# browserdotsys/vecchio

Measured on NVIDIA B200. Metric: Mpaths/s, higher is better.
Workload: dtype f32

## Files before the change

### include/vecchio_gpu.h

```cpp
#ifndef VECCHIO_GPU_H
#define VECCHIO_GPU_H

#include <stddef.h>
#include <stdint.h>

#ifdef __cplusplus
extern "C" {
#endif

#define VK_API_VERSION 1u

typedef enum vk_status {
    VK_OK = 0,
    VK_ERR_INVALID = -1,
    VK_ERR_NO_DEVICE = -2,
    VK_ERR_CUDA = -3,
    VK_ERR_UNSUPPORTED = -4,
    VK_ERR_NO_SCENE = -5,
    VK_ERR_OOM = -6
} vk_status;


typedef uint32_t vk_ref;

// ... 135 lines not shown
    float origin[3];
    float lower_left_corner[3];
    float horizontal[3];
    float vertical[3];
    float u[3], v[3], w[3];
    float lens_radius;
    float time0, time1;
} vk_camera;

enum { VK_VARIANT_AUTO = 0, VK_VARIANT_MEGAKERNEL = 1, VK_VARIANT_WAVEFRONT = 2, VK_VARIANT_STAGED = 3, VK_VARIANT_WARPQ = 4,
       VK_VARIANT_STEPQ = 5 };
enum {
    VK_FLAG_STRICT_MATH = 1u,
    VK_FLAG_FORCE_BVH = 2u,
    VK_FLAG_LEGACY_SCATTER = 4u,
    VK_FLAG_SKY_BACKGROUND = 8u
};

typedef struct vk_render_params {
    uint32_t width, height;
    uint32_t spp;
    uint32_t spp_begin;
    uint32_t spp_count;
    uint32_t max_depth;
    uint64_t seed;
    float background[3];
    uint32_t variant;
    uint32_t flags;
} vk_render_params;

typedef struct vk_stats {
    uint64_t paths;
    uint64_t rays;
    uint64_t dropped_samples;
    float ms_kernels;
    float ms_total;
    uint32_t variant;
    uint32_t launches;
    uint64_t node_visits;
    uint64_t prim_tests;
} vk_stats;

typedef struct vk_ray {
    float origin[3];
    float direction[3];
    float time;
    float tmin, tmax;
} vk_ray;

typedef struct vk_hit {
    vk_ref prim;
    uint32_t face;
    uint32_t mat;
    uint32_t front;
    float t;
    float p[3];
    float normal[3];
    float u, v;
    uint32_t _pad;
} vk_hit;

#define VK_MEDIUM_XI_SLOTS 8

typedef struct vk_ctx vk_ctx;

int vk_create(int device, vk_ctx** out);
void vk_destroy(vk_ctx* ctx);
const char* vk_last_error(const vk_ctx* ctx);

int vk_scene_upload(vk_ctx* ctx, const vk_scene_desc* scene);

typedef struct vk_scene_info {
    uint32_t flat_entries;
    uint32_t flat_segments;
    uint32_t flat_subtrees;
    uint32_t simple;
    uint32_t wide_nodes;
    uint32_t wide_levels_world;
    uint32_t wide_levels_instance;
    uint32_t stack_need;
    uint32_t dynamic_megakernel;
    uint32_t flat_boxes;
    uint32_t flat_direct;
} vk_scene_info;
int vk_scene_check(const vk_scene_desc* scene, vk_scene_info* info, char* err, size_t err_len);

int vk_render(vk_ctx* ctx, const vk_camera* cam, const vk_render_params* params,
              float* out_rgb, float* out_sumsq, vk_stats* stats);

int vk_render_rgb8(vk_ctx* ctx, const vk_camera* cam, const vk_render_params* params,
                   uint8_t* out_rgb8, vk_stats* stats);

int vk_render_frames(vk_ctx* ctx, const vk_camera* cams, uint32_t n_frames, const vk_render_params* params,
                     float* out_rgb, vk_stats* stats);
int vk_render_frames_rgb8(vk_ctx* ctx, const vk_camera* cams, uint32_t n_frames, const vk_render_params* params,
                          uint8_t* out_rgb8, vk_stats* stats);

int vk_render_adaptive(vk_ctx* ctx, const vk_camera* cam, const vk_render_params* params,
                       uint32_t pass_spp, float max_error,
                       float* out_rgb, uint32_t* out_spp, vk_stats* stats);
int vk_render_adaptive_rgb8(vk_ctx* ctx, const vk_camera* cam, const vk_render_params* params,
                            uint32_t pass_spp, float max_error,
                            uint8_t* out_rgb8, uint32_t* out_spp, vk_stats* stats);

int vk_render_frames_adaptive(vk_ctx* ctx, const vk_camera* cams, uint32_t n_frames, const vk_render_params* params,
                              uint32_t pass_spp, float max_error,
                              float* out_rgb, uint32_t* out_spp, vk_stats* stats);
int vk_render_frames_adaptive_rgb8(vk_ctx* ctx, const vk_camera* cams, uint32_t n_frames, const vk_render_params* params,
                                   uint32_t pass_spp, float max_error,
                                   uint8_t* out_rgb8, uint32_t* out_spp, vk_stats* stats);

typedef struct vk_adaptive_target {
    uint32_t spp;
    uint32_t min_spp;
    float max_error;
} vk_adaptive_target;
typedef struct vk_adaptive_session vk_adaptive_session;


int vk_adaptive_begin(vk_ctx* ctx, const vk_camera* cams, uint32_t n_frames, const vk_render_params* params,
                      uint32_t pass_spp, vk_adaptive_session** out);

#define VK_SHARD_RUN 32
int vk_adaptive_begin_shard(vk_ctx* ctx, const vk_camera* cams, uint32_t n_frames, const vk_render_params* params,
                            uint32_t pass_spp, uint32_t shard, uint32_t n_shards, vk_adaptive_session** out);

int vk_adaptive_refine(vk_adaptive_session* session, const vk_adaptive_target* target, vk_stats* stats);

int vk_adaptive_read(vk_adaptive_session* session, float* out_rgb, uint32_t* out_spp, float* out_error);
int vk_adaptive_read_rgb8(vk_adaptive_session* session, uint8_t* out_rgb8, uint32_t* out_spp, float* out_error);

int vk_adaptive_export(vk_adaptive_session* session, int64_t* sums, uint64_t* squares, uint32_t* counts,
                       vk_adaptive_target* reached);
int vk_adaptive_import(vk_adaptive_session* session, const int64_t* sums, const uint64_t* squares, const uint32_t* counts,
                       const vk_adaptive_target* reached);

uint32_t vk_adaptive_variant(const vk_adaptive_session* session);

void vk_adaptive_destroy(vk_adaptive_session* session);

int vk_render_device(vk_ctx* ctx, const vk_camera* cam, const vk_render_params* params,
                     float* d_sum, float* d_sumsq, vk_stats* stats);

int vk_finalize_device(vk_ctx* ctx, const float* d_sum, float* d_rgb, size_t n_floats,
                       uint32_t spp);

int vk_set_stream(vk_ctx* ctx, void* stream);

int vk_flush_stats(vk_ctx* ctx, vk_stats* stats);

typedef struct vk_multi vk_multi;
int vk_multi_create(const int* devices, int n_devices, vk_multi** out);
void vk_multi_destroy(vk_multi* m);
const char* vk_multi_last_error(const vk_multi* m);
int vk_multi_device_count(const vk_multi* m);
int vk_multi_scene_upload(vk_multi* m, const vk_scene_desc* scene);
int vk_multi_render(vk_multi* m, const vk_camera* cam, const vk_render_params* params, float* out_rgb, float* out_sumsq,
                    vk_stats* stats);
int vk_multi_render_rgb8(vk_multi* m, const vk_camera* cam, const vk_render_params* params, uint8_t* out_rgb8,
                         vk_stats* stats);
int vk_multi_render_frames_rgb8(vk_multi* m, const vk_camera* cams, uint32_t n_frames, const vk_render_params* params,
                                uint8_t* out_rgb8, vk_stats* stats);

typedef struct vk_multi_adaptive_session vk_multi_adaptive_session;
int vk_multi_adaptive_begin(vk_multi* m, const vk_camera* cams, uint32_t n_frames, const vk_render_params* params,
                            uint32_t pass_spp, vk_multi_adaptive_session** out);
// ... 45 lines not shown
```

### vecchio_b200/_abi.py

```python
import ctypes as C

VK_API_VERSION = 1
VK_OK = 0
VK_ERR_INVALID, VK_ERR_NO_DEVICE, VK_ERR_CUDA, VK_ERR_UNSUPPORTED, VK_ERR_NO_SCENE, VK_ERR_OOM = -1, -2, -3, -4, -5, -6

VK_T_NONE, VK_T_NODE, VK_T_SPHERE, VK_T_MSPHERE, VK_T_RECT, VK_T_BOX, VK_T_XFORM, VK_T_MEDIUM = range(8)
VK_VARIANT_AUTO, VK_VARIANT_MEGAKERNEL, VK_VARIANT_WAVEFRONT, VK_VARIANT_STAGED, VK_VARIANT_WARPQ, VK_VARIANT_STEPQ = 0, 1, 2, 3, 4, 5
VK_FLAG_STRICT_MATH = 1
VK_FLAG_FORCE_BVH = 2
VK_FLAG_LEGACY_SCATTER = 4
VK_FLAG_SKY_BACKGROUND = 8
VK_MEDIUM_XI_SLOTS = 8
VK_EVAL_BOUNCE, VK_EVAL_BOUNCE_LEGACY, VK_EVAL_TEXTURE, VK_EVAL_LIGHTS_PDF, VK_EVAL_LIGHT_RANDOM = range(5)
VK_M_LAMBERTIAN, VK_M_METAL, VK_M_DIELECTRIC, VK_M_DIFFUSE_LIGHT, VK_M_ISOTROPIC, VK_M_SPECDIFFUSE = range(6)
VK_TEX_SOLID, VK_TEX_CHECKER, VK_TEX_IMAGE, VK_TEX_NOISE = range(4)
VK_RECT_FLIP = 0x100


def ref_type(r):
    return (int(r) >> 28) & 0xF


def ref_index(r):
    return int(r) & 0x0FFFFFFF
# ... 1 lines not shown

class vk_node(C.Structure):
    _fields_ = [("bb_min", C.c_float * 3), ("left", C.c_uint32), ("bb_max", C.c_float * 3), ("right", C.c_uint32)]


class vk_sphere(C.Structure):
    _fields_ = [("center", C.c_float * 3), ("radius", C.c_float)]


class vk_msphere(C.Structure):
    _fields_ = [("center0", C.c_float * 3), ("radius", C.c_float), ("center1", C.c_float * 3), ("time0", C.c_float),
                ("time1", C.c_float), ("mat", C.c_uint32), ("_pad", C.c_uint32 * 2)]


class vk_rect(C.Structure):
    _fields_ = [("c0", C.c_float), ("c1", C.c_float), ("d0", C.c_float), ("d1", C.c_float), ("k", C.c_float),
                ("axes", C.c_uint32), ("mat", C.c_uint32), ("_pad", C.c_uint32)]


class vk_box(C.Structure):
    _fields_ = [("box_min", C.c_float * 3), ("mat", C.c_uint32), ("box_max", C.c_float * 3), ("_pad", C.c_uint32)]


class vk_xform(C.Structure):
    _fields_ = [("kind", C.c_uint32), ("child", C.c_uint32), ("_pad0", C.c_uint32 * 2), ("a", C.c_float),
                ("b", C.c_float), ("c", C.c_float), ("_pad1", C.c_uint32)]


class vk_medium(C.Structure):
    _fields_ = [("boundary", C.c_uint32), ("neg_inv_density", C.c_float), ("mat", C.c_uint32), ("_pad", C.c_uint32)]


class vk_material(C.Structure):
    _fields_ = [("type", C.c_uint32), ("tex", C.c_uint32), ("param", C.c_float), ("aux", C.c_uint32)]


class vk_texture(C.Structure):
    _fields_ = [("type", C.c_uint32), ("w", C.c_uint32 * 3)]


class vk_perlin(C.Structure):
    _fields_ = [("ranvec", (C.c_float * 3) * 256), ("perm_x", C.c_uint8 * 256), ("perm_y", C.c_uint8 * 256),
                ("perm_z", C.c_uint8 * 256)]


class vk_scene_desc(C.Structure):
    _fields_ = [
        ("api_version", C.c_uint32), ("root", C.c_uint32),
        ("nodes", C.POINTER(vk_node)), ("n_nodes", C.c_uint32),
        ("spheres", C.POINTER(vk_sphere)), ("sphere_mat", C.POINTER(C.c_uint32)), ("n_spheres", C.c_uint32),
        ("mspheres", C.POINTER(vk_msphere)), ("n_mspheres", C.c_uint32),
        ("rects", C.POINTER(vk_rect)), ("n_rects", C.c_uint32),
        ("boxes", C.POINTER(vk_box)), ("n_boxes", C.c_uint32),
        ("xforms", C.POINTER(vk_xform)), ("n_xforms", C.c_uint32),
        ("media", C.POINTER(vk_medium)), ("n_media", C.c_uint32),
        ("lights", C.POINTER(C.c_uint32)), ("n_lights", C.c_uint32),
        ("materials", C.POINTER(vk_material)), ("n_materials", C.c_uint32),
        ("textures", C.POINTER(vk_texture)), ("n_textures", C.c_uint32),
        ("texels", C.POINTER(C.c_uint8)), ("n_texel_bytes", C.c_uint64),
        ("perlins", C.POINTER(vk_perlin)), ("n_perlins", C.c_uint32),
    ]


class vk_camera(C.Structure):
    _fields_ = [("origin", C.c_float * 3), ("lower_left_corner", C.c_float * 3), ("horizontal", C.c_float * 3),
                ("vertical", C.c_float * 3), ("u", C.c_float * 3), ("v", C.c_float * 3), ("w", C.c_float * 3),
                ("lens_radius", C.c_float), ("time0", C.c_float), ("time1", C.c_float)]


class vk_render_params(C.Structure):
    _fields_ = [("width", C.c_uint32), ("height", C.c_uint32), ("spp", C.c_uint32), ("spp_begin", C.c_uint32),
                ("spp_count", C.c_uint32), ("max_depth", C.c_uint32), ("seed", C.c_uint64),
                ("background", C.c_float * 3), ("variant", C.c_uint32), ("flags", C.c_uint32)]


class vk_stats(C.Structure):
    _fields_ = [("paths", C.c_uint64), ("rays", C.c_uint64), ("dropped_samples", C.c_uint64),
                ("ms_kernels", C.c_float), ("ms_total", C.c_float), ("variant", C.c_uint32), ("launches", C.c_uint32),
                ("node_visits", C.c_uint64), ("prim_tests", C.c_uint64)]


class vk_scene_info(C.Structure):
    _fields_ = [(n, C.c_uint32) for n in ("flat_entries", "flat_segments", "flat_subtrees", "simple", "wide_nodes", "wide_levels_world",
                                          "wide_levels_instance", "stack_need", "dynamic_megakernel", "flat_boxes", "flat_direct")]


class vk_ray(C.Structure):
    _fields_ = [("origin", C.c_float * 3), ("direction", C.c_float * 3), ("time", C.c_float), ("tmin", C.c_float),
                ("tmax", C.c_float)]


class vk_hit(C.Structure):
    _fields_ = [("prim", C.c_uint32), ("face", C.c_uint32), ("mat", C.c_uint32), ("front", C.c_uint32),
                ("t", C.c_float), ("p", C.c_float * 3), ("normal", C.c_float * 3), ("u", C.c_float), ("v", C.c_float),
                ("_pad", C.c_uint32)]


assert C.sizeof(vk_node) == 32 and C.sizeof(vk_sphere) == 16 and C.sizeof(vk_msphere) == 48
assert C.sizeof(vk_rect) == 32 and C.sizeof(vk_box) == 32 and C.sizeof(vk_xform) == 32
assert C.sizeof(vk_medium) == 16 and C.sizeof(vk_material) == 16 and C.sizeof(vk_texture) == 16
assert C.sizeof(vk_camera) == 96 and C.sizeof(vk_ray) == 36 and C.sizeof(vk_hit) == 56

import numpy as _np

RAY_DTYPE = _np.dtype([("origin", "<f4", 3), ("direction", "<f4", 3), ("time", "<f4"), ("tmin", "<f4"), ("tmax", "<f4")])
HIT_DTYPE = _np.dtype([("prim", "<u4"), ("face", "<u4"), ("mat", "<u4"), ("front", "<u4"), ("t", "<f4"),
                       ("p", "<f4", 3), ("normal", "<f4", 3), ("u", "<f4"), ("v", "<f4"), ("_pad", "<u4")])
EVAL_DTYPE = _np.dtype([("op", "<u4"), ("index", "<u4"), ("ray_o", "<f4", 3), ("ray_d", "<f4", 3), ("ray_time", "<f4"),
                        ("p", "<f4", 3), ("normal", "<f4", 3), ("t", "<f4"), ("u", "<f4"), ("v", "<f4"), ("front", "<u4"),
                        ("dir", "<f4", 3), ("xi", "<u4", 5),
                        ("alive", "<u4"), ("valid", "<u4"), ("out_o", "<f4", 3), ("out_d", "<f4", 3), ("out_time", "<f4"),
                        ("beta", "<f4", 3), ("L", "<f4", 3), ("value", "<f4")])
assert RAY_DTYPE.itemsize == 36 and HIT_DTYPE.itemsize == 56 and EVAL_DTYPE.itemsize == 43 * 4


class vk_adaptive_target(C.Structure):
    _fields_ = [("spp", C.c_uint32), ("min_spp", C.c_uint32), ("max_error", C.c_float)]
```

### vecchio_b200/csrc/vk_api.cu

```cuda
#include <chrono>
#include <cstdio>
#include <cstdlib>
#include <cstring>
#include <functional>
#include <string>
#include <thread>
#include <vector>

#include <cub/device/device_select.cuh>
#include <thrust/iterator/counting_iterator.h>

#include "vk_internal.h"
#include "vk_relayout.h"

using namespace vkhost;

struct vk_ctx {
    int device = 0;
    int sm_count = 0;
    int clock_khz = 0;
    char name[128] = {0};
    cudaStream_t stream = nullptr;
    cudaStream_t own_stream = nullptr;
    uint64_t launches = 0;
    uint64_t paths = 0;
    cudaEvent_t ev0 = nullptr, ev1 = nullptr, ev2 = nullptr;
    std::string err;
    std::vector<void*> scene_allocs;
    char* arena = nullptr;
    size_t arena_cap = 0, arena_used = 0, arena_need = 0;
    cudaEvent_t ev_chunk[4] = {nullptr, nullptr, nullptr, nullptr};
    DScene scene{};
    FlatProgram flat{};
    bool has_scene = false;
    uint32_t n_nodes = 0;
    uint32_t n_materials = 0, n_textures = 0, n_media = 0;
    size_t wnodes_bytes = 0;
    size_t l2_persist_max = 0, l2_window_max = 0;
    bool has_specdiffuse = false;
    bool simple_scene = false;
    bool one_rect_light = false;
    unsigned long long* debug = nullptr;
    unsigned long long* counters = nullptr;
    float* partial = nullptr;
    size_t partial_floats = 0;
    float* sq_stack = nullptr;
    size_t sq_stack_floats = 0;
    uint32_t stack_need = 0, levels_sub = 0;
    float* frame = nullptr;
    size_t frame_floats = 0;
    float* pinned = nullptr;
    size_t pinned_floats = 0;
    DCamera* cams = nullptr;
    size_t cams_cap = 0;
    std::vector<DCamera> cams_host;
    vk_adaptive_session* oneshot = nullptr;
    uint64_t scene_gen = 0;
    WfState wf{};
    void* wf_block = nullptr;
    uint32_t* wf_host_counts = nullptr;
};

static thread_local std::string g_create_err;
extern "C" {
static void adaptive_free(vk_adaptive_session* s);
}

static int fail(vk_ctx* c, int code, const std::string& msg) {
    if (c) c->err = msg;
    else g_create_err = msg;
    return code;
}
#define CU(ctx, call)                                                                                                  \
    do {                                                                                                               \
        cudaError_t e_ = (call);                                                                                       \
        if (e_ != cudaSuccess)                                                                                         \
            return fail(ctx, e_ == cudaErrorMemoryAllocation ? VK_ERR_OOM : VK_ERR_CUDA,                               \
                        std::string(#call) + ": " + cudaGetErrorString(e_));                                           \
    } while (0)

__global__ void k_acc_to_sum(const unsigned long long* __restrict__ acc, const double* __restrict__ accsq, size_t n,
                             float* __restrict__ sum, float* __restrict__ sumsq) {
    const size_t i = (size_t)blockIdx.x * blockDim.x + threadIdx.x;
    if (i >= n) return;
    sum[i] = (float)((double)(long long)acc[i] * VK_ACC_INV_SCALE);
    if (sumsq) sumsq[i] = (float)accsq[i];
}
struct SumsOverSpp {
    static constexpr bool counted = false;
    const float* __restrict__ sum;
    float spp;
    __device__ float mean(size_t j) const { return sum[j] / spp; }
};
struct AccOverCount {
    static constexpr bool counted = true;
    const unsigned long long* __restrict__ acc;
    const uint32_t* __restrict__ nspp;
    __device__ float mean(size_t j) const { return (float)((double)(long long)acc[j] * VK_ACC_INV_SCALE) / (float)nspp[j / 3]; }
};
__device__ __forceinline__ size_t flip_rows(size_t i, uint32_t width, uint32_t height, uint32_t per) {
    const size_t row_len = (size_t)width * per, frame = row_len * height, f = i / frame, k = i - f * frame, row = k / row_len;
    return f * frame + (height - 1 - row) * row_len + (k - row * row_len);
}
template <class Src> __global__ void k_finalize(Src src, float* __restrict__ rgb, size_t n) {
    const size_t i = (size_t)blockIdx.x * blockDim.x + threadIdx.x;
    if (i < n) rgb[i] = src.mean(i);
}
template <class Src>
__global__ void k_to_color(Src src, uint8_t* __restrict__ out, uint32_t* __restrict__ spp_out, uint32_t width, uint32_t height, uint32_t n_frames) {
    const size_t i = (size_t)blockIdx.x * blockDim.x + threadIdx.x;
    if (i >= (size_t)width * height * 3 * n_frames) return;
    const size_t j = flip_rows(i, width, height, 3);
    float v = sqrtf(src.mean(j));
    v = v < 0.0f ? 0.0f : (v > 0.999f ? 0.999f : v);
    out[i] = (uint8_t)__float2uint_rz(256.0f * v);
    if constexpr (Src::counted)
        if (spp_out && i % 3 == 0) spp_out[i / 3] = src.nspp[j / 3];
}
__device__ __forceinline__ bool shard_owns(uint32_t p, uint32_t shard, uint32_t n_shards) {
    return (p / VK_SHARD_RUN) % n_shards == shard;
}
__global__ void k_shard_list(uint32_t* list, uint32_t n_owned, uint32_t shard, uint32_t n_shards) {
    const uint32_t i = blockIdx.x * blockDim.x + threadIdx.x;
    if (i < n_owned) list[i] = ((i / VK_SHARD_RUN) * n_shards + shard) * VK_SHARD_RUN + i % VK_SHARD_RUN;
// ... 243 lines not shown
    for (uint32_t i = 0; i < d->n_materials; ++i) {
        bool uv;
        if (mats[i].type == VK_M_SPECDIFFUSE)
            uv = (d->materials[mats[i].tex].type != VK_M_DIELECTRIC && v.tex_has_image(d->materials[mats[i].tex].tex, 0)) ||
                 (d->materials[mats[i].aux].type != VK_M_DIELECTRIC && v.tex_has_image(d->materials[mats[i].aux].tex, 0));
        else
            uv = mats[i].type != VK_M_DIELECTRIC && v.tex_has_image(mats[i].tex, 0);
        if (uv) mats[i].aux |= VKD_MAT_NEEDS_UV;
    }
    std::vector<float4> pvec((size_t)d->n_perlins * 256);
    std::vector<uint8_t> pperm((size_t)d->n_perlins * 768);
    for (uint32_t p = 0; p < d->n_perlins; ++p) {
        for (int k = 0; k < 256; ++k)
            pvec[(size_t)p * 256 + k] = make_float4(d->perlins[p].ranvec[k][0], d->perlins[p].ranvec[k][1], d->perlins[p].ranvec[k][2], 0.f);
        std::memcpy(&pperm[(size_t)p * 768], d->perlins[p].perm_x, 256);
        std::memcpy(&pperm[(size_t)p * 768 + 256], d->perlins[p].perm_y, 256);
        std::memcpy(&pperm[(size_t)p * 768 + 512], d->perlins[p].perm_z, 256);
    }

    std::vector<uint8_t> pcls;
    uint32_t cls_base[8] = {0, 0, 0, 0, 0, 0, 0, 0};
    {
        auto cls_of = [&](uint32_t mat) -> uint8_t {
            const uint32_t t = mat < d->n_materials ? d->materials[mat].type : (uint32_t)VK_M_LAMBERTIAN;
            return t == VK_M_DIFFUSE_LIGHT ? 0 : t == VK_M_DIELECTRIC ? 1 : t == VK_M_METAL ? 2 : 3;
        };
        cls_base[VK_T_SPHERE] = (uint32_t)pcls.size();
        for (uint32_t i = 0; i < d->n_spheres; ++i) pcls.push_back(cls_of(d->sphere_mat[i]));
        cls_base[VK_T_MSPHERE] = (uint32_t)pcls.size();
        for (uint32_t i = 0; i < d->n_mspheres; ++i) pcls.push_back(cls_of(d->mspheres[i].mat));
        cls_base[VK_T_RECT] = (uint32_t)pcls.size();
        for (uint32_t i = 0; i < d->n_rects; ++i) pcls.push_back(cls_of(d->rects[i].mat));
        cls_base[VK_T_BOX] = (uint32_t)pcls.size();
        for (uint32_t i = 0; i < d->n_boxes; ++i) pcls.push_back(cls_of(d->boxes[i].mat));
        cls_base[VK_T_MEDIUM] = (uint32_t)pcls.size();
        for (uint32_t i = 0; i < d->n_media; ++i) pcls.push_back(cls_of(d->media[i].mat));
        pcls.push_back(3);
    }

    DScene s{};
    int rc;
#define UP(field, type, src, n)                                                                                        \
    if ((rc = upload<type>(c, (const type*)(src), (n), (const type**)&s.field)) != VK_OK) {                            \
        free_scene(c);                                                                                                 \
        return rc;                                                                                                     \
    }
    UP(wnodes, float4, wnodes.data(), wnodes.size())
    UP(nodes, float4, nodes.data(), (size_t)d->n_nodes * 2)
    UP(spheres, float4, d->spheres, d->n_spheres)
    UP(sphere_mat, uint32_t, d->sphere_mat, d->n_spheres)
    UP(mspheres, float4, d->mspheres, (size_t)d->n_mspheres * 3)
    UP(rects, float4, d->rects, (size_t)d->n_rects * 2)
    UP(boxes, float4, d->boxes, (size_t)d->n_boxes * 2)
    UP(xforms, float4, d->xforms, (size_t)d->n_xforms * 2)
    UP(media, float4, d->media, d->n_media)
    UP(media_plan, float4, R.media_plan.data(), R.media_plan.size())
    UP(lights, uint32_t, d->lights, d->n_lights)
    UP(materials, uint4, mats.data(), d->n_materials)
    UP(textures, uint4, d->textures, d->n_textures)
    UP(texels, uint8_t, d->texels, (size_t)d->n_texel_bytes)
    UP(perlin_vec, float4, pvec.data(), pvec.size())
    UP(perlin_perm, uint8_t, pperm.data(), pperm.size())
    UP(flat_shade, float4, R.flat_shade.data(), R.flat_shade.size())
    UP(prim_cls, uint8_t, pcls.data(), pcls.size())
#undef UP
    for (int t = 0; t < 8; ++t) s.cls_base[t] = cls_base[t];
    s.root = d->root;
    s.n_lights = d->n_lights;
    s.has_media = d->n_media > 0;
    s.light0_a = s.light0_b = make_float4(0.f, 0.f, 0.f, 0.f);
    if (d->n_lights >= 1 && VK_REF_TYPE(d->lights[0]) == VK_T_RECT) {
        static_assert(sizeof(vk_rect) == 2 * sizeof(float4), "device rect record");
        std::memcpy(&s.light0_a, &d->rects[VK_REF_INDEX(d->lights[0])], 2 * sizeof(float4));
    }
    CU(c, cudaStreamSynchronize(c->stream));
    c->scene = s;
    c->n_nodes = d->n_nodes;
    c->n_materials = d->n_materials;
    c->n_textures = d->n_textures;
    c->n_media = d->n_media;
    c->wnodes_bytes = wnodes.size() * sizeof(float4);
    c->has_specdiffuse = R.has_specdiffuse;
    c->simple_scene = R.simple;
    c->one_rect_light = d->n_lights == 1 && VK_REF_TYPE(d->lights[0]) == VK_T_RECT && !(d->rects[VK_REF_INDEX(d->lights[0])].axes & VK_RECT_FLIP);
    c->stack_need = R.stack_need;
    c->levels_sub = R.levels_sub;
    c->flat = R.flat;
    c->has_scene = true;
    return VK_OK;
}

extern "C" int vk_flush_stats(vk_ctx* c, vk_stats* stats);

static int wf_ensure(vk_ctx* c) {
    uint32_t n = 1u << 19;
    if (const char* e = std::getenv("VECCHIO_WF_SLOTS")) {
        const long v = std::atol(e);
        if (v >= 1024 && v <= (1l << 26)) n = (uint32_t)v;
    }
    n = (n + 255u) & ~255u;
    if (c->wf_block && c->wf.n_slots == n) return VK_OK;
    if (c->wf_block) cudaFree(c->wf_block);
    c->wf_block = nullptr;
    c->wf = WfState{};
    const size_t per_slot = 16 * 5 + 4 * VKW_CLASSES;
    const size_t tail = 256;
    CU(c, cudaMalloc(&c->wf_block, per_slot * n + tail));
    char* p = (char*)c->wf_block;
    auto take = [&](size_t bytes) { char* q = p; p += bytes; return q; };
    c->wf.ray_o = (float4*)take(16ull * n);
    c->wf.ray_d = (float4*)take(16ull * n);
    c->wf.beta = (float4*)take(16ull * n);
    c->wf.unit = (uint4*)take(16ull * n);
    c->wf.hit = (uint4*)take(16ull * n);
    c->wf.queue = (uint32_t*)take(4ull * VKW_CLASSES * n);
    c->wf.qcount = (uint32_t*)take(64);
    c->wf.unit_head = (unsigned long long*)take(64);
    c->wf.n_slots = n;
    if (!c->wf_host_counts) CU(c, cudaMallocHost((void**)&c->wf_host_counts, 64));
    return VK_OK;
}

static int wf_render(vk_ctx* c, bool strict, const FlatProgram* flat, const DCamera& dc, const RenderArgs& a, const RenderBuffers& b,
                     uint32_t* launches) {
    int rc = wf_ensure(c);
    if (rc != VK_OK) return rc;
    WfState w = c->wf;
    w.n_pixels = a.width * a.height;
    w.n_units = (unsigned long long)w.n_pixels * a.spp_count;
    const unsigned long long head0 = w.n_units < w.n_slots ? w.n_units : w.n_slots;
    CU(c, cudaMemsetAsync(w.qcount, 0, 64, c->stream));
    CU(c, cudaMemcpyAsync(w.unit_head, &head0, sizeof(head0), cudaMemcpyHostToDevice, c->stream));
    CU(c, strict ? vkstrict::launch_wf_generate(dc, a, w, c->stream) : vkfast::launch_wf_generate(dc, a, w, c->stream));
    ++*launches;
    const unsigned long long min_iters = ((unsigned long long)w.n_pixels * a.spp_count + w.n_slots - 1) / w.n_slots;
    unsigned long long next_check = min_iters > 8 ? min_iters : 8;
    const unsigned long long max_iters = (min_iters + 2) * (unsigned long long)(a.max_depth ? a.max_depth : 1) + 64;
    for (unsigned long long it = 0;; ++it) {
        if (it > max_iters) {
            cudaStreamSynchronize(c->stream);
            return fail(c, VK_ERR_CUDA, "wavefront: the slot pool did not drain (internal error)");
        }
        const uint32_t set = (uint32_t)(it & 1u);
        CU(c, strict ? vkstrict::launch_wf_extend(c->scene, flat, a, w, b, set, c->stream)
                     : vkfast::launch_wf_extend(c->scene, flat, a, w, b, set, c->stream));
        CU(c, strict ? vkstrict::launch_wf_shade(c->scene, dc, a, w, b, set, c->stream)
                     : vkfast::launch_wf_shade(c->scene, dc, a, w, b, set, c->stream));
        *launches += flat ? 2 : 3;
        if (it + 1 >= next_check) {
            CU(c, cudaMemcpyAsync(c->wf_host_counts, w.qcount + set * VKW_CLASSES, VKW_CLASSES * sizeof(uint32_t), cudaMemcpyDeviceToHost, c->stream));
            CU(c, cudaStreamSynchronize(c->stream));
            const uint32_t live = c->wf_host_counts[0] + c->wf_host_counts[1] + c->wf_host_counts[2] + c->wf_host_counts[3];
            if (live == 0) break;
            next_check = it + 1 + (live == w.n_slots ? 32 : 8);
        }
    }
    return VK_OK;
}


static uint32_t choose_variant(const vk_ctx* c, const vk_render_params* P, uint32_t n_frames = 1) {
    if (P->variant != VK_VARIANT_AUTO) return P->variant;
    const bool flat = c->flat.n && !(P->flags & VK_FLAG_FORCE_BVH);
    const char* e = std::getenv("VECCHIO_AUTO");
    if (e && !std::strcmp(e, "staged")) return flat && c->flat.n_bvh == 0 ? (uint32_t)VK_VARIANT_STAGED : (uint32_t)VK_VARIANT_MEGAKERNEL;
    if (e && !std::strcmp(e, "warpq")) return (uint32_t)VK_VARIANT_WARPQ;
// ... 82 lines not shown
    if (!legacy && c->scene.n_lights == 0)
        return fail(c, VK_ERR_INVALID, who + ": empty light list (the reference panics: choose().unwrap(), src/hittable.rs:431); only VK_FLAG_LEGACY_SCATTER renders without lights");
    if (const int rc = check_variant(c, who, variant, n_frames, list); rc != VK_OK) return rc;
    const bool l0 = !strict && !legacy && c->one_rect_light && !c->has_specdiffuse && !std::getenv("VECCHIO_NO_LIGHT0");
    CU(c, strict ? vkstrict::megakernel_occupancy(flat != nullptr, c->scene.has_media, legacy, &bps, &bt)
          : l0   ? vkfast_l0::megakernel_occupancy(flat != nullptr, c->scene.has_media, legacy, &bps, &bt)
                 : vkfast::megakernel_occupancy(flat != nullptr, c->scene.has_media, legacy, &bps, &bt));
    if (bps < 1) bps = 1;
    R->legacy = legacy;
    R->l0 = l0;
    R->flat = flat;
    R->grid = c->sm_count * bps;
    R->resident_warps = (uint32_t)R->grid * (uint32_t)bt / 32u;
    if (variant == VK_VARIANT_STEPQ && flat && flat->n_bvh == 0) variant = VK_VARIANT_WARPQ;
    R->variant = variant;
    return VK_OK;
}

static int upload_cams(vk_ctx* c, const vk_camera* cams, uint32_t n_frames) {
    if (c->cams_cap < n_frames) {
        if (c->cams) cudaFree(c->cams);
        c->cams = nullptr;
        c->cams_cap = 0;
        CU(c, cudaMalloc((void**)&c->cams, n_frames * sizeof(DCamera)));
        c->cams_cap = n_frames;
    }
    c->cams_host.resize(n_frames);
    for (uint32_t f = 0; f < n_frames; ++f) c->cams_host[f] = to_dcam(cams + f);
    CU(c, cudaMemcpyAsync(c->cams, c->cams_host.data(), n_frames * sizeof(DCamera), cudaMemcpyHostToDevice, c->stream));
    return VK_OK;
}

static int launch_pass(vk_ctx* c, const RenderPlan& R, const vk_camera* cam, const vk_render_params* P, uint32_t spp_begin, uint32_t count,
                       const RenderBuffers& b, uint32_t n_frames, const ListArgs* ls, uint32_t* launches) {
    const bool strict = R.strict, legacy = R.legacy, l0 = R.l0;
    const FlatProgram* flat = R.flat;
    const uint32_t variant = R.variant;
    RenderArgs a{};
    a.width = P->width;
    a.height = P->height;
    a.spp_begin = spp_begin;
    a.spp_count = count;
    a.max_depth = P->max_depth;
    a.seed_lo = (uint32_t)P->seed;
    a.seed_hi = (uint32_t)(P->seed >> 32);
    a.background = make_float3(P->background[0], P->background[1], P->background[2]);
    a.flags = P->flags;
    a.tiles_x = (P->width + 7) / 8;
    a.tiles_y = (P->height + 3) / 4;
    if (ls) {
        a.tiles_x = (ls->n + 31) / 32;
        a.tiles_y = 1;
    }
    const uint32_t n_tiles = a.tiles_x * a.tiles_y * (ls ? 1u : n_frames);
    uint32_t n_chunks = (48u * R.resident_warps + n_tiles - 1) / n_tiles;
    if (n_chunks > count) n_chunks = count;
    if (n_chunks < 1) n_chunks = 1;
    a.chunk_spp = (count + n_chunks - 1) / n_chunks;
    a.n_chunks = (count + a.chunk_spp - 1) / a.chunk_spp;

    CU(c, cudaMemsetAsync(c->counters + 2, 0, sizeof(unsigned long long), c->stream));
    const DCamera dc = to_dcam(cam);
    auto run = [&](const auto& dom) -> int {
        if (variant == VK_VARIANT_STEPQ) {
            const bool inst = c->levels_sub != 0u;
            uint32_t glevels = 0;
            const size_t words = strict ? vkstrict::stepq_stack_words(c->stack_need, inst, c->sm_count, &glevels)
                                        : vkfast::stepq_stack_words(c->stack_need, inst, c->sm_count, &glevels);
            if (words) {
                const int rc = ensure(c, &c->sq_stack, &c->sq_stack_floats, words);
                if (rc != VK_OK) return rc;
            }
            CU(c, cudaMemsetAsync(c->counters + 2, 0, sizeof(unsigned long long), c->stream));
            CU(c, cudaMemsetAsync(c->counters + 5, 0, sizeof(unsigned long long), c->stream));
            CU(c, strict ? vkstrict::launch_stepq(c->scene, dc, a, b, c->counters + 2, (uint32_t*)c->sq_stack, glevels, inst, c->sm_count, legacy, c->stream, dom)
                  : l0   ? vkfast_l0::launch_stepq(c->scene, dc, a, b, c->counters + 2, (uint32_t*)c->sq_stack, glevels, inst, c->sm_count, legacy, c->stream, dom)
                         : vkfast::launch_stepq(c->scene, dc, a, b, c->counters + 2, (uint32_t*)c->sq_stack, glevels, inst, c->sm_count, legacy, c->stream, dom));
            *launches += 1;
        } else if (variant == VK_VARIANT_WARPQ) {
            CU(c, cudaMemsetAsync(c->counters + 2, 0, sizeof(unsigned long long), c->stream));
            CU(c, cudaMemsetAsync(c->counters + 5, 0, sizeof(unsigned long long), c->stream));
            const FlatProgram* sflat = flat;
            const bool simple = !strict && !legacy && sflat && sflat->n_bvh == 0 && c->simple_scene && !std::getenv("VECCHIO_NO_SIMPLE");
            CU(c, strict   ? vkstrict::launch_warpq(c->scene, sflat, dc, a, b, c->counters + 2, c->sm_count, legacy, c->stream, dom)
                  : simple ? vkfast_simple::launch_warpq(c->scene, sflat, dc, a, b, c->counters + 2, c->sm_count, legacy, c->stream, dom)
                  : l0     ? vkfast_l0::launch_warpq(c->scene, sflat, dc, a, b, c->counters + 2, c->sm_count, legacy, c->stream, dom)
                           : vkfast::launch_warpq(c->scene, sflat, dc, a, b, c->counters + 2, c->sm_count, legacy, c->stream, dom));
            *launches += 1;
        } else if (variant == VK_VARIANT_WAVEFRONT) {
            uint32_t n = 0;
            int rc = wf_render(c, strict, flat, dc, a, b, &n);
            if (rc != VK_OK) return rc;
            *launches += n;
        } else if (variant == VK_VARIANT_STAGED) {
            CU(c, cudaMemsetAsync(c->counters + 5, 0xFF, 2 * sizeof(unsigned long long), c->stream));
            CU(c, cudaMemsetAsync(c->counters + 7, 0, sizeof(unsigned long long), c->stream));
            CU(c, cudaMemsetAsync(c->counters + 2, 0, sizeof(unsigned long long), c->stream));
            const FlatProgram* sflat = flat && flat->n_bvh == 0 ? flat : nullptr;
            const bool simple = !strict && sflat && c->simple_scene && !std::getenv("VECCHIO_NO_SIMPLE");
            CU(c, strict   ? vkstrict::launch_staged(c->scene, sflat, dc, a, b, c->counters + 2, c->sm_count, c->stream)
                  : simple ? vkfast_simple::launch_staged(c->scene, sflat, dc, a, b, c->counters + 2, c->sm_count, c->stream)
                           : vkfast::launch_staged(c->scene, sflat, dc, a, b, c->counters + 2, c->sm_count, c->stream));
            *launches += 1;
        } else if (!flat && !legacy && use_dynamic_megakernel(c)) {
            CU(c, cudaMemsetAsync(c->counters + 2, 0, sizeof(unsigned long long), c->stream));
            CU(c, strict ? vkstrict::launch_megakernel_dyn(c->scene, dc, a, b, c->counters + 2, c->sm_count, c->stream, dom)
                  : l0   ? vkfast_l0::launch_megakernel_dyn(c->scene, dc, a, b, c->counters + 2, c->sm_count, c->stream, dom)
                         : vkfast::launch_megakernel_dyn(c->scene, dc, a, b, c->counters + 2, c->sm_count, c->stream, dom));
            *launches += 1;
        } else {
            CU(c, strict ? vkstrict::launch_megakernel(c->scene, flat, dc, a, b, R.grid, legacy, c->stream, dom)
                  : l0   ? vkfast_l0::launch_megakernel(c->scene, flat, dc, a, b, R.grid, legacy, c->stream, dom)
                         : vkfast::launch_megakernel(c->scene, flat, dc, a, b, R.grid, legacy, c->stream, dom));
            *launches += 1;
        }
        return VK_OK;
    };
    if (n_frames == 1) return ls ? run(*ls) : run(OneFrame{});
    int rc = upload_cams(c, cam, n_frames);
    if (rc != VK_OK) return rc;
    const FrameArgs fr{c->cams, n_frames, P->width * P->height};
    return ls ? run(FrameListArgs{fr, *ls}) : run(fr);
}

static int render_into(vk_ctx* c, const vk_camera* cam, const vk_render_params* P, float* d_sum, float* d_sumsq, vk_stats* stats,
                       bool acc_only = false, bool want_sq = false, uint32_t n_frames = 1) {
    if (!c) return VK_ERR_INVALID;
    int rc = check_render(c, "render", cam, n_frames, P);
    if (rc != VK_OK) return rc;
    if (!d_sum && !acc_only) return fail(c, VK_ERR_INVALID, "render: null argument");
    if (!acc_only) want_sq = d_sumsq != nullptr;
    const uint32_t count = P->spp_count ? P->spp_count : P->spp - P->spp_begin;
    CU(c, cudaSetDevice(c->device));
    RenderPlan R;
    if ((rc = plan_render(c, "render", P, n_frames, false, &R)) != VK_OK) return rc;

    const size_t plane = (size_t)P->width * P->height * 3 * n_frames;
    RenderBuffers b{};
    b.counters = c->counters;
    b.debug = c->debug;
    {
        rc = ensure(c, &c->partial, &c->partial_floats, plane * (want_sq ? 4 : 2));
        if (rc != VK_OK) return rc;
        b.acc = (unsigned long long*)c->partial;
        b.accsq = want_sq ? (double*)(c->partial + plane * 2) : nullptr;
        CU(c, cudaMemsetAsync(c->partial, 0, plane * (want_sq ? 4 : 2) * sizeof(float), c->stream));
    }
    apply_l2_window(c);
    CU(c, cudaEventRecord(c->ev0, c->stream));
    uint32_t launches = 0;
    if ((rc = launch_pass(c, R, cam, P, P->spp_begin, count, b, n_frames, nullptr, &launches)) != VK_OK) return rc;
    if (!acc_only) {
        k_acc_to_sum<<<(unsigned)((plane + 255) / 256), 256, 0, c->stream>>>(b.acc, b.accsq, plane, d_sum, d_sumsq);
        ++launches;
    }
    CU(c, cudaGetLastError());
    CU(c, cudaEventRecord(c->ev1, c->stream));
    c->launches += launches;
    c->paths += (uint64_t)P->width * P->height * count * n_frames;
    if (stats) {
        rc = vk_flush_stats(c, stats);
        if (rc != VK_OK) return rc;
        CU(c, cudaEventElapsedTime(&stats->ms_kernels, c->ev0, c->ev1));
        stats->ms_total = stats->ms_kernels;
        stats->variant = R.variant;
    }
    return VK_OK;
}

int vk_render_device(vk_ctx* c, const vk_camera* cam, const vk_render_params* P, float* d_sum, float* d_sumsq, vk_stats* stats) {
// ... 1101 lines not shown
```

### vecchio_b200/csrc/vk_device.cuh

```cuda
#pragma once
#include <math_constants.h>

#include "vk_internal.h"

#ifndef VK_STRICT
#define VK_STRICT 0
#endif
#ifndef VK_SIMPLE
#define VK_SIMPLE 0
#endif
#ifndef VK_LIGHT0
#define VK_LIGHT0 0
#endif
#if VK_STRICT
#define VK_NS vkstrict
#elif VK_SIMPLE
#define VK_NS vkfast_simple
#elif VK_LIGHT0
#define VK_NS vkfast_l0
#else
#define VK_NS vkfast
#endif

namespace VK_NS {
// ... 485 lines not shown
        float3 to = T.co, td = T.cd, tinv = T.cinv;
        uint32_t leaf = ref, inst = T.cur_inst;
        if (type == VK_T_XFORM) {
            leaf = chain_down(sc, ref, to, td) | (ref & VKD_DUP);
            inst = ref & ~VKD_DUP;
            if (VKD_TYPE(leaf) == VK_T_NODE) {
                T.stack[T.sp++] = VKD_T_EXIT << 28;
                T.co = to;
                T.cd = td;
                T.cinv = rcp3(td);
                T.cur_inst = inst;
                T.ref = leaf & ~VKD_DUP;
                T.enter = true;
                return;
            }
            tinv = rcp3(td);
        }
        float t;
        uint32_t face = 0;
        bool hit;
        ++tc.prims;
        if (MEDIA && VKD_TYPE(leaf) == VK_T_MEDIUM) hit = medium_t(sc, leaf, to, td, time, tmin, T.best.t, xi, t);
        else hit = leaf_t(sc, leaf, to, td, tinv, time, tmin, T.best.t, t, face);
        if (hit) {
            T.best.t = t;
            T.best.prim = leaf & ~VKD_DUP;
            T.best.inst = inst;
            T.best.face = face;
        }
    }
    T.ref = trav_pop(T);
}

template <bool MEDIA>
VKD TraceHit trace(const DScene& sc, float3 o, float3 d, float time, float tmin, float tmax, const MediumXi& xi, TraceCounters& tc) {
    Trav T;
    trav_init(T, sc, o, d, tmax);
#pragma unroll 1
    for (;;) {
#pragma unroll 1
        while (trav_at_node(T)) trav_node_step(T, sc, tmin, tc);
        if (T.ref == VKD_DONE) break;
        trav_prim_step<MEDIA>(T, sc, o, d, time, tmin, xi, tc);
    }
    return T.best;
}

#if VK_STRICT
#define VKF_PLANE_T(K, O, D, I) (((K) - (O)) / (D))
#else
#define VKF_PLANE_T(K, O, D, I) (((K) - (O)) * (I))
#endif
template <int AX, bool BOX_SIDE>
VKD void flat_rects(const FlatProgram& P, uint32_t i0, uint32_t i1, float3 co, float3 cd, float3 ci, float tmin, float& best_t,
                    uint32_t& best_hit) {
#pragma unroll 1
    for (uint32_t i = i0; i < i1; ++i) {
        const float4 bd = P.rects[i].bounds;
        const float k = P.rects[i].k;
        float tt, a, b;
        if (AX == 0) {
            tt = VKF_PLANE_T(k, co.z, cd.z, ci.z);
            a = co.x + tt * cd.x;
            b = co.y + tt * cd.y;
        } else if (AX == 1) {
            tt = VKF_PLANE_T(k, co.y, cd.y, ci.y);
            a = co.x + tt * cd.x;
            b = co.z + tt * cd.z;
        } else {
            tt = VKF_PLANE_T(k, co.x, cd.x, ci.x);
            a = co.y + tt * cd.y;
            b = co.z + tt * cd.z;
        }
        bool hit = !(tt < tmin || tt > best_t) && !(a < bd.x || a > bd.y || b < bd.z || b > bd.w);
        if (BOX_SIDE) hit = hit && tt < best_t;
        if (hit) {
            best_t = tt;
            best_hit = P.rects[i].hit;
        }
    }
}
#if !VK_STRICT
template <int K>
VKD void flat_boxes_k(const FlatProgram& P, uint32_t i0, uint32_t i1, const float3 (&co)[K], const float3 (&ci)[K], float tmin,
                      float (&best_t)[K], uint32_t (&best_hit)[K]) {
#pragma unroll 1
    for (uint32_t i = i0; i < i1; ++i) {
        const float4 mn = P.boxes[i].mn, mx = P.boxes[i].mx;
        const uint32_t hz = __float_as_uint(mn.w), hy = __float_as_uint(mx.w) & 0xFFFFu, hx = __float_as_uint(mx.w) >> 16;
#pragma unroll
        for (int q = 0; q < K; ++q) {
            const float x0 = (mn.x - co[q].x) * ci[q].x, x1 = (mx.x - co[q].x) * ci[q].x;
            const float y0 = (mn.y - co[q].y) * ci[q].y, y1 = (mx.y - co[q].y) * ci[q].y;
            const float z0 = (mn.z - co[q].z) * ci[q].z, z1 = (mx.z - co[q].z) * ci[q].z;
            const float nx = fminf(x0, x1), ny = fminf(y0, y1), nz = fminf(z0, z1);
            const float fx = fmaxf(x0, x1), fy = fmaxf(y0, y1), fz = fmaxf(z0, z1);
            const float t_near = fmaxf(fmaxf(nx, ny), nz), t_far = fminf(fminf(fx, fy), fz);
            const bool enter = t_near >= tmin;
            const float t = enter ? t_near : t_far;
            const bool hit = (t_near <= t_far) & (t >= tmin) & (t < best_t[q]);
            const bool on_z = (enter ? nz : fz) == t, on_y = (enter ? ny : fy) == t;
            const float at_max = on_z ? z1 : (on_y ? y1 : x1);
            const uint32_t id = (on_z ? hz : (on_y ? hy : hx)) + (at_max == t ? 0u : 1u);
            best_t[q] = hit ? t : best_t[q];
            best_hit[q] = hit ? id : best_hit[q];
        }
    }
}
#endif
template <bool MEDIA>
VKD TraceHit trace_flat(const DScene& sc, const FlatProgram& P, float3 o, float3 d, float time, float tmin, float tmax,
                        const MediumXi& xi, TraceCounters& tc) {
    float best_t = tmax;
    uint32_t best_hit = 0xFFFFFFFFu;
    TraceHit sub;
    sub.t = tmax;
    sub.prim = VK_REF_NONE;
    sub.inst = 0;
    sub.face = 0;
    const uint32_t n_segs = P.n_segs;
    tc.prims += P.n;
#pragma unroll 1
    for (uint32_t s = 0; s < n_segs; ++s) {
        const FlatSeg& g = P.segs[s];
        float3 co = o, cd = d;
#pragma unroll 1
        for (uint32_t k = g.op0; k < g.op1; ++k) {
            const uint32_t kind = P.ops[k].kind;
            if (kind == VKF_OP_TRANSLATE) co = co - f3(P.ops[k].a, P.ops[k].b, P.ops[k].c);
            else {
                rot_fwd(kind, P.ops[k].a, P.ops[k].b, co);
                rot_fwd(kind, P.ops[k].a, P.ops[k].b, cd);
            }
        }
        const float3 ci = rcp3(cd);
        flat_rects<0, false>(P, g.rect0[0], g.rect1[0], co, cd, ci, tmin, best_t, best_hit);
        flat_rects<1, false>(P, g.rect0[1], g.rect1[1], co, cd, ci, tmin, best_t, best_hit);
        flat_rects<2, false>(P, g.rect0[2], g.rect1[2], co, cd, ci, tmin, best_t, best_hit);
#if VK_STRICT
        flat_rects<0, true>(P, g.rect0[3], g.rect1[3], co, cd, ci, tmin, best_t, best_hit);
        flat_rects<1, true>(P, g.rect0[4], g.rect1[4], co, cd, ci, tmin, best_t, best_hit);
        flat_rects<2, true>(P, g.rect0[5], g.rect1[5], co, cd, ci, tmin, best_t, best_hit);
#else
        {
            const float3 co1[1] = {co}, ci1[1] = {ci};
            float bt1[1] = {best_t};
            uint32_t bh1[1] = {best_hit};
            flat_boxes_k<1>(P, g.box0, g.box1, co1, ci1, tmin, bt1, bh1);
            best_t = bt1[0];
            best_hit = bh1[0] == 0xFFFFFFFFu ? bh1[0] : VKF_HIT_INDEX(bh1[0]);
        }
#endif
#pragma unroll 1
        for (uint32_t i = g.sph0; i < g.sph1; ++i) {
            float tt;
            if (sphere_t(f3(P.spheres[i].a), P.spheres[i].a.w, co, cd, tmin, best_t, tt)) {
                best_t = tt;
                best_hit = P.spheres[i].hit;
            }
        }
#pragma unroll 1
        for (uint32_t i = g.msph0; i < g.msph1; ++i) {
            float tt;
            if (sphere_t(msphere_center(P.spheres[i].a, P.spheres[i].b, P.spheres[i].time1, time), P.spheres[i].a.w, co, cd, tmin, best_t, tt)) {
                best_t = tt;
                best_hit = P.spheres[i].hit;
            }
        }
        if (MEDIA) {
#pragma unroll 1
            for (uint32_t i = g.med0; i < g.med1; ++i) {
                float tt;
                if (medium_t(sc, P.hits[i].prim, co, cd, time, tmin, best_t, xi, tt)) {
                    best_t = tt;
                    best_hit = i;
                }
            }
        }
#pragma unroll 1
        for (uint32_t i = g.bvh0; i < g.bvh1; ++i) {
            Trav T;
            T.sp = 0;
            T.co = co;
            T.cd = cd;
            T.cinv = ci;
            T.cur_inst = P.seg_inst[s];
            T.best.t = best_t;
            T.best.prim = VK_REF_NONE;
            T.best.inst = 0;
            T.best.face = 0;
            T.ref = P.bvh[i];
            T.enter = true;
#pragma unroll 1
            for (;;) {
#pragma unroll 1
                while (trav_at_node(T)) trav_node_step(T, sc, tmin, tc);
                if (T.ref == VKD_DONE) break;
                trav_prim_step<false>(T, sc, o, d, time, tmin, xi, tc);
            }
            if (T.best.prim != VK_REF_NONE) {
                best_t = T.best.t;
                sub = T.best;
                best_hit = 0xFFFFFFFEu;
            }
        }
    }
    TraceHit best;
    best.t = best_t;
    best.prim = VK_REF_NONE;
    best.inst = 0;
    best.face = 0;
    if (best_hit == 0xFFFFFFFEu) return sub;
    if (best_hit != 0xFFFFFFFFu) {
        best.prim = P.hits[best_hit].prim & ~VKD_DUP;
        best.inst = P.hits[best_hit].inst;
        best.face = P.hits[best_hit].face;
    }
    return best;
}

template <int K, int AX, bool BOX_SIDE>
VKD void flat_rects_k(const FlatProgram& P, uint32_t i0, uint32_t i1, const float3 (&co)[K], const float3 (&cd)[K], const float3 (&ci)[K],
                      float tmin, float (&best_t)[K], uint32_t (&best_hit)[K]) {
#pragma unroll 1
    for (uint32_t i = i0; i < i1; ++i) {
        const float4 bd = P.rects[i].bounds;
        const float k = P.rects[i].k;
        const uint32_t id = P.rects[i].hitc;
#pragma unroll
        for (int q = 0; q < K; ++q) {
            float tt, a, b;
            if (AX == 0) {
                tt = VKF_PLANE_T(k, co[q].z, cd[q].z, ci[q].z);
                a = co[q].x + tt * cd[q].x;
                b = co[q].y + tt * cd[q].y;
            } else if (AX == 1) {
                tt = VKF_PLANE_T(k, co[q].y, cd[q].y, ci[q].y);
                a = co[q].x + tt * cd[q].x;
                b = co[q].z + tt * cd[q].z;
            } else {
                tt = VKF_PLANE_T(k, co[q].x, cd[q].x, ci[q].x);
                a = co[q].y + tt * cd[q].y;
                b = co[q].z + tt * cd[q].z;
            }
            bool miss = (a < bd.x) | (a > bd.y) | (b < bd.z) | (b > bd.w) | (tt < tmin);
            miss = miss | (tt > best_t[q]);
            if (BOX_SIDE) miss = miss | !(tt < best_t[q]);
            best_t[q] = miss ? best_t[q] : tt;
            best_hit[q] = miss ? best_hit[q] : id;
        }
    }
}
#if !VK_STRICT
#ifndef VKF_INLINE_MEDIA
#define VKF_INLINE_MEDIA 1
#endif
VKD bool flat_medium_box(const FlatMedium& fm, uint32_t ref, float3 o, float3 d, float tmin, float tmax, const MediumXi& xi, float& t) {
    float3 bo = o, bd = d;
    if (__float_as_uint(fm.mx.w) & 2u) {
        const float* m = fm.aff;
        bo = f3(fmaf(m[0], o.x, fmaf(m[1], o.y, fmaf(m[2], o.z, m[9]))), fmaf(m[3], o.x, fmaf(m[4], o.y, fmaf(m[5], o.z, m[10]))),
                fmaf(m[6], o.x, fmaf(m[7], o.y, fmaf(m[8], o.z, m[11]))));
        bd = f3(fmaf(m[0], d.x, fmaf(m[1], d.y, m[2] * d.z)), fmaf(m[3], d.x, fmaf(m[4], d.y, m[5] * d.z)),
                fmaf(m[6], d.x, fmaf(m[7], d.y, m[8] * d.z)));
    }
    const float3 binv = rcp3(bd);
    const float3 oi = f3(-bo.x * binv.x, -bo.y * binv.y, -bo.z * binv.z);
    const float x0 = fmaf(fm.mn.x, binv.x, oi.x), x1 = fmaf(fm.mx.x, binv.x, oi.x);
    const float y0 = fmaf(fm.mn.y, binv.y, oi.y), y1 = fmaf(fm.mx.y, binv.y, oi.y);
    const float z0 = fmaf(fm.mn.z, binv.z, oi.z), z1 = fmaf(fm.mx.z, binv.z, oi.z);
    const float t_near = fmaxf(fmaxf(fminf(x0, x1), fminf(y0, y1)), fminf(z0, z1));
    const float t_far = fminf(fminf(fmaxf(x0, x1), fmaxf(y0, y1)), fmaxf(z0, z1));
    if (!(t_near <= t_far)) return false;
    float t1 = (t_near >= -CUDART_INF_F) ? t_near : t_far;
    if (!(t1 >= -CUDART_INF_F && t1 < CUDART_INF_F)) return false;
    const float lo = t1 + 0.0001f;
    float t2 = (t_near >= lo) ? t_near : t_far;
    if (!(t2 >= lo && t2 < CUDART_INF_F)) return false;
    if (t1 < tmin) t1 = tmin;
    if (t2 > tmax) t2 = tmax;
    if (t1 >= t2) return false;
    if (t1 < 0.0f) t1 = 0.0f;
    const float ray_length = sqrtf(length2(d));
    const float distance_inside_boundary = (t2 - t1) * ray_length;
    const float hit_distance = fm.mn.w * logf(xi.get(VKD_INDEX(ref), (ref & VKD_DUP) ? 1u : 0u));
    if (hit_distance > distance_inside_boundary) return false;
    t = t1 + hit_distance / ray_length;
    return true;
}
#endif
template <int K, bool MEDIA, bool HYBRID>
VKD void flat_segment_k(const DScene& sc, const FlatProgram& P, const FlatSeg& g, uint32_t s, const float3 (&o)[K], const float3 (&d)[K],
                        const float3 (&co)[K], const float3 (&cd)[K], const float (&time)[K], const bool (&live)[K], float tmin,
                        const MediumXi (&xi)[K], float (&best_t)[K], uint32_t (&best_hit)[K], TraceHit* sub, TraceCounters* tc) {
    float3 ci[K];
#pragma unroll
    for (int q = 0; q < K; ++q) ci[q] = rcp3(cd[q]);
    flat_rects_k<K, 0, false>(P, g.rect0[0], g.rect1[0], co, cd, ci, tmin, best_t, best_hit);
    flat_rects_k<K, 1, false>(P, g.rect0[1], g.rect1[1], co, cd, ci, tmin, best_t, best_hit);
    flat_rects_k<K, 2, false>(P, g.rect0[2], g.rect1[2], co, cd, ci, tmin, best_t, best_hit);
#if VK_STRICT
    flat_rects_k<K, 0, true>(P, g.rect0[3], g.rect1[3], co, cd, ci, tmin, best_t, best_hit);
    flat_rects_k<K, 1, true>(P, g.rect0[4], g.rect1[4], co, cd, ci, tmin, best_t, best_hit);
    flat_rects_k<K, 2, true>(P, g.rect0[5], g.rect1[5], co, cd, ci, tmin, best_t, best_hit);
#else
    flat_boxes_k<K>(P, g.box0, g.box1, co, ci, tmin, best_t, best_hit);
#endif
#pragma unroll 1
    for (uint32_t i = g.sph0; i < g.sph1; ++i) {
        const float4 sp = P.spheres[i].a;
        const uint32_t id = P.spheres[i].hitc;
#pragma unroll
        for (int q = 0; q < K; ++q) {
            float tt;
            if (sphere_t(f3(sp), sp.w, co[q], cd[q], tmin, best_t[q], tt)) {
                best_t[q] = tt;
                best_hit[q] = id;
            }
        }
    }
#if !VK_SIMPLE
#pragma unroll 1
    for (uint32_t i = g.msph0; i < g.msph1; ++i) {
#pragma unroll
        for (int q = 0; q < K; ++q) {
            float tt;
            if (sphere_t(msphere_center(P.spheres[i].a, P.spheres[i].b, P.spheres[i].time1, time[q]), P.spheres[i].a.w, co[q], cd[q], tmin, best_t[q], tt)) {
                best_t[q] = tt;
                best_hit[q] = P.spheres[i].hitc;
            }
        }
    }
#endif
    if (MEDIA) {
#pragma unroll 1
        for (uint32_t i = g.med0; i < g.med1; ++i) {
#if !VK_STRICT && VKF_INLINE_MEDIA
            const FlatMedium& fm = P.fmed[P.seg_fm0[s] + (i - g.med0)];
            const bool inline_box = (__float_as_uint(fm.mx.w) & 1u) != 0u;
#endif
#pragma unroll
            for (int q = 0; q < K; ++q) {
                float tt;
                bool hit;
#if !VK_STRICT && VKF_INLINE_MEDIA
                if (inline_box) hit = live[q] && flat_medium_box(fm, P.hits[i].prim, co[q], cd[q], tmin, best_t[q], xi[q], tt);
                else
#endif
                    hit = live[q] && medium_t(sc, P.hits[i].prim, co[q], cd[q], time[q], tmin, best_t[q], xi[q], tt);
                if (hit) {
                    best_t[q] = tt;
                    best_hit[q] = VKF_HITC(i, P.hits[i].cls, P.hits[i].inst);
                }
            }
        }
    }
    if (HYBRID) {
#pragma unroll 1
        for (uint32_t i = g.bvh0; i < g.bvh1; ++i) {
#pragma unroll
            for (int q = 0; q < K; ++q) {
                Trav T;
                T.sp = 0;
                T.co = co[q];
                T.cd = cd[q];
                T.cinv = ci[q];
                T.cur_inst = P.seg_inst[s];
                T.best.t = best_t[q];
                T.best.prim = VK_REF_NONE;
                T.best.inst = 0;
                T.best.face = 0;
                T.ref = live[q] ? P.bvh[i] : VKD_DONE;
                T.enter = true;
#pragma unroll 1
                for (;;) {
#pragma unroll 1
                    while (trav_at_node(T)) trav_node_step(T, sc, tmin, *tc);
                    if (T.ref == VKD_DONE) break;
                    trav_prim_step<false>(T, sc, o[q], d[q], time[q], tmin, xi[q], *tc);
                }
                if (T.best.prim != VK_REF_NONE) {
                    best_t[q] = T.best.t;
                    sub[q] = T.best;
                    best_hit[q] = 0xFFFFFFFEu;
                }
            }
        }
    }
}
#ifndef VKF_PEEL_WORLD
#define VKF_PEEL_WORLD 1
#endif
template <int K, bool MEDIA, bool HYBRID = false>
VKD void trace_flat_k(const DScene& sc, const FlatProgram& P, const float3 (&o)[K], const float3 (&d)[K], const float (&time)[K],
                      const bool (&live)[K], float tmin, const MediumXi (&xi)[K], float (&best_t)[K], uint32_t (&best_hit)[K],
                      TraceHit* sub = nullptr, TraceCounters* tc = nullptr) {
#pragma unroll
    for (int q = 0; q < K; ++q) {
        best_t[q] = CUDART_INF_F;
        best_hit[q] = 0xFFFFFFFFu;
    }
    const uint32_t n_segs = P.n_segs;
#if !VK_STRICT && VKF_PEEL_WORLD
    if constexpr (!MEDIA) {
    flat_segment_k<K, MEDIA, HYBRID>(sc, P, P.segs[0], 0u, o, d, o, d, time, live, tmin, xi, best_t, best_hit, sub, tc);
#pragma unroll 1
    for (uint32_t s = 1; s < n_segs; ++s) {
        const FlatSeg& g = P.segs[s];
        float3 co[K], cd[K];
        {
            const float* m = P.seg_affine[s];
            const float r00 = m[0], r01 = m[1], r02 = m[2], r10 = m[3], r11 = m[4], r12 = m[5], r20 = m[6], r21 = m[7], r22 = m[8];
            const float t0 = m[9], t1 = m[10], t2 = m[11];
#pragma unroll
            for (int q = 0; q < K; ++q) {
                const float3 wo = o[q], wd = d[q];
                co[q] = f3(fmaf(r00, wo.x, fmaf(r01, wo.y, fmaf(r02, wo.z, t0))), fmaf(r10, wo.x, fmaf(r11, wo.y, fmaf(r12, wo.z, t1))),
                           fmaf(r20, wo.x, fmaf(r21, wo.y, fmaf(r22, wo.z, t2))));
                cd[q] = f3(fmaf(r00, wd.x, fmaf(r01, wd.y, r02 * wd.z)), fmaf(r10, wd.x, fmaf(r11, wd.y, r12 * wd.z)),
                           fmaf(r20, wd.x, fmaf(r21, wd.y, r22 * wd.z)));
            }
        }
        flat_segment_k<K, MEDIA, HYBRID>(sc, P, g, s, o, d, co, cd, time, live, tmin, xi, best_t, best_hit, sub, tc);
    }
    return;
    }
#endif
    {
#pragma unroll 1
    for (uint32_t s = 0; s < n_segs; ++s) {
        const FlatSeg& g = P.segs[s];
        float3 co[K], cd[K];
#pragma unroll
        for (int q = 0; q < K; ++q) {
            co[q] = o[q];
            cd[q] = d[q];
        }
#if VK_STRICT
#pragma unroll 1
        for (uint32_t k = g.op0; k < g.op1; ++k) {
            const uint32_t kind = P.ops[k].kind;
            const float pa = P.ops[k].a, pb = P.ops[k].b, pc = P.ops[k].c;
#pragma unroll
            for (int q = 0; q < K; ++q) {
                if (kind == VKF_OP_TRANSLATE) co[q] = co[q] - f3(pa, pb, pc);
                else {
                    rot_fwd(kind, pa, pb, co[q]);
                    rot_fwd(kind, pa, pb, cd[q]);
                }
            }
        }
#else
        if (g.op1 != g.op0) {
            const float* m = P.seg_affine[s];
            const float r00 = m[0], r01 = m[1], r02 = m[2], r10 = m[3], r11 = m[4], r12 = m[5], r20 = m[6], r21 = m[7], r22 = m[8];
            const float t0 = m[9], t1 = m[10], t2 = m[11];
#pragma unroll
            for (int q = 0; q < K; ++q) {
                const float3 wo = co[q], wd = cd[q];
                co[q] = f3(fmaf(r00, wo.x, fmaf(r01, wo.y, fmaf(r02, wo.z, t0))), fmaf(r10, wo.x, fmaf(r11, wo.y, fmaf(r12, wo.z, t1))),
                           fmaf(r20, wo.x, fmaf(r21, wo.y, fmaf(r22, wo.z, t2))));
                cd[q] = f3(fmaf(r00, wd.x, fmaf(r01, wd.y, r02 * wd.z)), fmaf(r10, wd.x, fmaf(r11, wd.y, r12 * wd.z)),
                           fmaf(r20, wd.x, fmaf(r21, wd.y, r22 * wd.z)));
            }
        }
#endif
        flat_segment_k<K, MEDIA, HYBRID>(sc, P, g, s, o, d, co, cd, time, live, tmin, xi, best_t, best_hit, sub, tc);
    }
    }
}

struct HitRecD {
    float3 p, normal;
    float t, u, v;
    uint32_t front, mat;
    uint4 m;
};

static __device__ __noinline__ float2 spherical_uv(float px, float py, float pz) {
    const float phi = atan2f(pz, px);
    const float theta = asinf(py);
    return make_float2(1.0f - ((phi + VK_PI) / (2.0f * VK_PI)), (theta + VK_PI / 2.0f) / VK_PI);
}
VKD void spherical(float3 p, float& u, float& v) {
    const float2 uv = spherical_uv(p.x, p.y, p.z);
    u = uv.x;
    v = uv.y;
}
VKD void set_face_normal(float3 dir, float3 outward, HitRecD& rec) {
    rec.front = dot3(dir, outward) < 0.0f ? 1u : 0u;
    rec.normal = rec.front ? outward : -outward;
}
VKD void rect_record(float4 bounds, float k, uint32_t axes, uint32_t flip, float3 o, float3 d, float t, bool want_uv,
                     HitRecD& rec) {
    (void)k;
    const uint32_t a0 = axes & 3u, a1 = (axes >> 2) & 3u, a2 = (axes >> 4) & 3u;
    rec.p = at(o, d, t);
    set_face_normal(d, f3(a2 == 0 ? 1.0f : 0.0f, a2 == 1 ? 1.0f : 0.0f, a2 == 2 ? 1.0f : 0.0f), rec);
    if (flip) rec.front ^= 1u;
    if (want_uv) {
        const float a = comp(o, a0) + t * comp(d, a0);
        const float b = comp(o, a1) + t * comp(d, a1);
        rec.u = (a - bounds.x) / (bounds.y - bounds.x);
        rec.v = (b - bounds.z) / (bounds.w - bounds.z);
    }
}
VKD void box_side(float3 mn, float3 mx, uint32_t face, float4& bounds, float& k, uint32_t& axes) {
    switch (face >> 1) {
    case 0: bounds = make_float4(mn.x, mx.x, mn.y, mx.y); k = (face & 1u) ? mn.z : mx.z; axes = 0u | (1u << 2) | (2u << 4); break;
    case 1: bounds = make_float4(mn.x, mx.x, mn.z, mx.z); k = (face & 1u) ? mn.y : mx.y; axes = 0u | (2u << 2) | (1u << 4); break;
    default: bounds = make_float4(mn.y, mx.y, mn.z, mx.z); k = (face & 1u) ? mn.x : mx.x; axes = 1u | (2u << 2) | (0u << 4); break;
    }
}
VKD void leaf_record(const DScene& sc, uint32_t ref, uint32_t face, float3 o, float3 d, float time, float t, bool always_uv,
                     HitRecD& rec) {
    const uint32_t i = VKD_INDEX(ref);
    rec.t = t;
    rec.u = 0.0f;
    rec.v = 0.0f;
    bool want_uv = always_uv;
#if VK_SIMPLE
    want_uv = false;
#endif
    switch (VKD_TYPE(ref)) {
    case VK_T_SPHERE:
#if !VK_SIMPLE
    case VK_T_MSPHERE:
#endif
    {
        float3 c;
        float radius;
        if (VK_SIMPLE || VKD_TYPE(ref) == VK_T_SPHERE) {
            const float4 s = __ldg(&sc.spheres[i]);
            c = f3(s);
            radius = s.w;
            rec.mat = __ldg(&sc.sphere_mat[i]);
        } else {
            const float4 m0 = __ldg(&sc.mspheres[3 * i]), m1 = __ldg(&sc.mspheres[3 * i + 1]), m2 = __ldg(&sc.mspheres[3 * i + 2]);
            c = msphere_center(m0, m1, m2.x, time);
            radius = m0.w;
            rec.mat = __float_as_uint(m2.y);
        }
        rec.m = __ldg(&sc.materials[rec.mat]);
        want_uv = !VK_SIMPLE && (want_uv || (rec.m.w & VKD_MAT_NEEDS_UV));
        rec.p = at(o, d, t);
        const float3 outward = (rec.p - c) / radius;
        set_face_normal(d, outward, rec);
        if (want_uv) spherical(outward, rec.u, rec.v);
        break;
    }
    case VK_T_RECT: {
        const float4 r0 = __ldg(&sc.rects[2 * i]), r1 = __ldg(&sc.rects[2 * i + 1]);
        const uint32_t axes = __float_as_uint(r1.y);
// ... 265 lines not shown
        const float3 direction = f3(s) - o;
        const float distance_squared = length2(direction);
        const Onb uvw = onb_from_w(direction);
        const float r1 = u01(x0), r2 = u01(x1);
        const float z = 1.0f + r2 * (sqrtf(1.0f - s.w * s.w / distance_squared) - 1.0f);
        float sn, cs;
        sincosf(2.0f * VK_PI * r1, &sn, &cs);
        const float x = cs * (1.0f - z * z), y = sn * (1.0f - z * z);
        return uvw.u * x + uvw.v * y + uvw.w * z;
    }
    case VK_T_BOX: {
        const float4 b0 = __ldg(&sc.boxes[2 * i]), b1 = __ldg(&sc.boxes[2 * i + 1]);
        const uint32_t f = min(5u, (uint32_t)(u01(x2) * 6.0f));
        if (f & 1u) return f3(1.0f, 0.0f, 0.0f);
        float4 bounds;
        float k;
        uint32_t axes;
        box_side(f3(b0), f3(b1), f, bounds, k, axes);
        return rect_random(bounds, k, axes, o, x0, x1);
    }
    default: return f3(1.0f, 0.0f, 0.0f);
    }
}
#endif
VKD float3 light_random(const DScene& sc, uint32_t ref, float3 o, uint32_t x0, uint32_t x1, uint32_t x2) {
    if (VKD_TYPE(ref) == VK_T_RECT) {
        const uint32_t i = VKD_INDEX(ref);
        const float4 r0 = __ldg(&sc.rects[2 * i]), r1 = __ldg(&sc.rects[2 * i + 1]);
        if (__float_as_uint(r1.y) & VK_RECT_FLIP) return f3(1.0f, 0.0f, 0.0f);
        return rect_random(r0, r1.x, __float_as_uint(r1.y), o, x0, x1);
    }
#if VK_SIMPLE
    (void)x2;
    return f3(1.0f, 0.0f, 0.0f);
#else
    return light_random_other(sc, ref, o, x0, x1, x2);
#endif
}
VKD float lights_pdf_value(const DScene& sc, float3 o, float3 v) {
#if VK_SIMPLE || VK_LIGHT0
    return 0.0f + 1.0f * rect_pdf_value(sc.light0_a, sc.light0_b.x, __float_as_uint(sc.light0_b.y), o, v);
#endif
    const float weight = 1.0f / (float)sc.n_lights;
    float sum = 0.0f;
#pragma unroll 1
    for (uint32_t l = 0; l < sc.n_lights; ++l) sum += weight * light_pdf_value(sc, __ldg(&sc.lights[l]), o, v);
    return sum;
}

static __device__ __noinline__ float2 camera_lens_disk(uint32_t pixel, uint32_t sample, uint32_t k0, uint32_t k1, float lens_radius) {
    const uint4 q = philox4x32_10(make_uint4(pixel, sample, 1u, 0u), make_uint2(k0, k1));
    const float rad = sqrtf(u01(q.x)) * lens_radius;
    float sn, cs;
    __sincosf(2.0f * VK_PI * u01(q.y), &sn, &cs);
    return make_float2(rad * cs, rad * sn);
}
VKD void camera_get_ray(const DCamera& cam, const PathRng& rng, uint32_t x, uint32_t y, uint32_t width, uint32_t height,
                        float3& o, float3& d, float& time) {
    const uint4 r = rng.block(0u, 0u);
    const float s = ((float)x + u01(r.x)) / (float)(width - 1);
    const float t = ((float)y + u01(r.y)) / (float)(height - 1);
    float3 offset = f3(0.0f, 0.0f, 0.0f);
    if (cam.lens_radius != 0.0f) {
        const float2 disk = camera_lens_disk(rng.pixel, rng.sample, rng.key.x, rng.key.y, cam.lens_radius);
        offset = cam.u * disk.x + cam.v * disk.y;
    }
    o = cam.origin + offset;
    d = cam.lower_left_corner + cam.horizontal * s + cam.vertical * t - cam.origin - offset;
    time = gen_range(r.z, cam.time0, cam.time1);
}

struct BounceXiPhilox {
    const PathRng& rng;
    uint32_t depth;
    VKD uint4 block0() const { return rng.block(depth, 0u); }
    VKD uint32_t spec() const { return rng.block(depth, 9u).x; }
};
struct BounceXiTable {
    uint4 r;
    uint32_t s;
    VKD uint4 block0() const { return r; }
    VKD uint32_t spec() const { return s; }
};
template <class XI>
VKD bool shade_xi(const DScene& sc, const HitRecD& rec, const XI& xi, float3& o, float3& d, float& time,
                  float3& beta, float3& L, bool& valid) {
    uint4 m = rec.m;
    uint32_t type = m.x;
    uint32_t spdf_type = type;
    float3 emitted = f3(0.0f, 0.0f, 0.0f);
    if (!VK_SIMPLE && !VK_LIGHT0 && type == VK_M_SPECDIFFUSE) {
        const uint32_t diffuse = m.w & ~VKD_MAT_NEEDS_UV;
        spdf_type = __ldg(&sc.materials[diffuse]).x;
        m = __ldg(&sc.materials[u01(xi.spec()) < __uint_as_float(m.z) ? m.y : diffuse]);
        type = m.x;
    } else if (type == VK_M_DIFFUSE_LIGHT) {
        if (rec.front) emitted = tex_value(sc, m.y, rec.u, rec.v, rec.p);
    }
    if (type == VK_M_DIFFUSE_LIGHT) {
        L = L + beta * emitted;
        return false;
    }
    const uint4 r = xi.block0();
    if (type == VK_M_DIELECTRIC) {
        const float ref_idx = __uint_as_float(m.z);
        const float etai_over_etat = rec.front ? 1.0f / ref_idx : ref_idx;
        const float3 unit_direction = unit_vector(d);
        const float cos_theta = fminf(dot3(-unit_direction, rec.normal), 1.0f);
        const float sin_theta = sqrtf(1.0f - cos_theta * cos_theta);
        float3 nd;
        if (etai_over_etat * sin_theta > 1.0f) nd = reflect(unit_direction, rec.normal);
        else if (u01(r.x) < schlick(cos_theta, etai_over_etat)) nd = reflect(unit_direction, rec.normal);
        else nd = refract(unit_direction, rec.normal, etai_over_etat);
        o = rec.p;
        d = nd;
        return true;
    }
    if (!VK_SIMPLE && type == VK_M_METAL) {
        const float fuzz = __uint_as_float(m.z);
        float3 nd = reflect(unit_vector(d), rec.normal);
        if (fuzz != 0.0f) nd = nd + random_in_unit_sphere(u01(r.x), u01(r.y), u01(r.z)) * fuzz;
        beta = beta * tex_value(sc, m.y, rec.u, rec.v, rec.p);
        o = rec.p;
        d = nd;
        time = 0.0f;
        return true;
    }
    const float3 attenuation = tex_value(sc, m.y, rec.u, rec.v, rec.p);
#if VK_STRICT
    const Onb uvw = onb_from_w(rec.normal);
    const float3 onb_w = uvw.w;
#else
    const float3 onb_w = unit_vector(rec.normal);
#endif
    float3 nd;
    if (u01(r.x) < 0.5f) {
#if VK_SIMPLE || VK_LIGHT0
        nd = rect_random(sc.light0_a, sc.light0_b.x, __float_as_uint(sc.light0_b.y), rec.p, r.y, r.z);
#else
        const uint32_t li = sc.n_lights > 1 ? min(sc.n_lights - 1u, (uint32_t)(u01(r.w) * (float)sc.n_lights)) : 0u;
        nd = light_random(sc, __ldg(&sc.lights[li]), rec.p, r.y, r.z, r.w * 0x9E3779B1u);
#endif
    } else {
        const float3 c = random_cosine_direction(u01(r.y), u01(r.z));
#if !VK_STRICT
        const Onb uvw = onb_from_w(rec.normal);
#endif
        nd = uvw.u * c.x + uvw.v * c.y + uvw.w * c.z;
    }
    const float3 und = unit_vector(nd);
    const float cos_w = dot3(und, onb_w);
    const float cosine_pdf = cos_w <= 0.0f ? 0.0f : cos_w / VK_PI;
    const float pdf = 0.5f * lights_pdf_value(sc, rec.p, nd) + 0.5f * cosine_pdf;
    float spdf = 0.0f;
    if (spdf_type == VK_M_LAMBERTIAN || spdf_type == VK_M_ISOTROPIC) {
        const float cos_n = dot3(rec.normal, und);
        spdf = cos_n < 0.0f ? 0.0f : cos_n / VK_PI;
    }
#if VK_STRICT
    const float3 w = f3(attenuation.x * spdf / pdf, attenuation.y * spdf / pdf, attenuation.z * spdf / pdf);
#else
    const float3 w = attenuation * (spdf / pdf);
#endif
    if (!finite3(w)) {
        valid = false;
        return false;
    }
    beta = beta * w;
    if (beta.x == 0.0f && beta.y == 0.0f && beta.z == 0.0f) return false;
    o = rec.p;
    d = nd;
    return true;
}
VKD bool shade(const DScene& sc, const HitRecD& rec, const PathRng& rng, uint32_t depth, float3& o, float3& d, float& time,
               float3& beta, float3& L, bool& valid) {
    const BounceXiPhilox xi = {rng, depth};
    return shade_xi(sc, rec, xi, o, d, time, beta, L, valid);
}

VKD void accumulate_sample(const RenderBuffers& buf, uint32_t pixel, float3 L) {
    unsigned long long* p = buf.acc + (size_t)pixel * 3u;
    const float lim = 4294967296.0f;
    if (L.x != 0.0f) atomicAdd(p + 0, (unsigned long long)__float2ll_rn(fminf(fmaxf(L.x, -lim), lim) * VK_ACC_SCALE));
    if (L.y != 0.0f) atomicAdd(p + 1, (unsigned long long)__float2ll_rn(fminf(fmaxf(L.y, -lim), lim) * VK_ACC_SCALE));
    if (L.z != 0.0f) atomicAdd(p + 2, (unsigned long long)__float2ll_rn(fminf(fmaxf(L.z, -lim), lim) * VK_ACC_SCALE));
    if (buf.accsq) {
        double* q = buf.accsq + (size_t)pixel * 3u;
        if (L.x != 0.0f) atomicAdd(q + 0, (double)L.x * (double)L.x);
        if (L.y != 0.0f) atomicAdd(q + 1, (double)L.y * (double)L.y);
        if (L.z != 0.0f) atomicAdd(q + 2, (double)L.z * (double)L.z);
    }
}
VKD void accumulate_square(unsigned long long* sq, uint32_t pixel, float3 L) {
    unsigned long long* q = sq + (size_t)pixel * 3u;
    const double cx = fminf(fabsf(L.x), VK_SQ_CLAMP), cy = fminf(fabsf(L.y), VK_SQ_CLAMP), cz = fminf(fabsf(L.z), VK_SQ_CLAMP);
    if (L.x != 0.0f) atomicAdd(q + 0, __double2ull_rn(cx * cx * (double)VK_SQ_SCALE));
    if (L.y != 0.0f) atomicAdd(q + 1, __double2ull_rn(cy * cy * (double)VK_SQ_SCALE));
    if (L.z != 0.0f) atomicAdd(q + 2, __double2ull_rn(cz * cz * (double)VK_SQ_SCALE));
}

VKD uint2 frame_key(const RenderArgs& a, uint32_t f) {
    const unsigned long long k = (((unsigned long long)a.seed_hi << 32) | a.seed_lo) + f;
    return make_uint2((uint32_t)k, (uint32_t)(k >> 32));
}
template <class D> VKD uint32_t dom_frames(const D&) { return 1u; }
VKD uint32_t dom_frames(const FrameArgs& fr) { return fr.n_frames; }
template <class D> VKD uint32_t dom_pixels(const D&, const RenderArgs& a) { return a.width * a.height; }
VKD uint32_t dom_pixels(const ListArgs& ls, const RenderArgs&) { return ls.n; }
VKD uint32_t dom_pixels(const FrameListArgs& fl, const RenderArgs&) { return fl.ls.n; }
template <class D> VKD uint32_t dom_list_pixel(const D&, uint32_t i) { return i; }
VKD uint32_t dom_list_pixel(const ListArgs& ls, uint32_t i) { return ls.list[i]; }
VKD uint32_t dom_list_pixel(const FrameListArgs& fl, uint32_t i) { return fl.ls.list[i]; }
template <class D, class T> VKD uint32_t dom_split_frame(const D&, T&, T) { return 0u; }
template <class T> VKD uint32_t dom_split_frame(const FrameArgs&, T& u, T per) {
    const uint32_t f = (uint32_t)(u / per);
    u -= (T)f * per;
    return f;
}
template <class D> VKD uint32_t dom_plane(const D&, uint32_t) { return 0u; }
VKD uint32_t dom_plane(const FrameArgs& fr, uint32_t f) { return f * fr.n_pix; }
template <class D> VKD const DCamera& dom_camera(const D&, const DCamera& cam, uint32_t) { return cam; }
VKD const DCamera& dom_camera(const FrameArgs& fr, const DCamera&, uint32_t f) { return fr.cams[f]; }
VKD const DCamera& dom_camera(const FrameListArgs& fl, const DCamera&, uint32_t f) { return fl.fr.cams[f]; }
template <class D> VKD void dom_frame_key(const D&, const RenderArgs&, uint32_t, PathRng&) {}
VKD void dom_frame_key(const FrameArgs&, const RenderArgs& a, uint32_t f, PathRng& rng) { rng.key = frame_key(a, f); }
template <class D> VKD void dom_slot_rng(const D&, const RenderArgs&, PathRng&) {}
VKD void dom_slot_rng(const FrameArgs& fr, const RenderArgs& a, PathRng& rng) {
    const uint32_t f = rng.pixel / fr.n_pix;
    rng.pixel = rng.pixel - f * fr.n_pix;
    rng.key = frame_key(a, f);
}
VKD void dom_slot_rng(const FrameListArgs& fl, const RenderArgs& a, PathRng& rng) { dom_slot_rng(fl.fr, a, rng); }
template <class D> struct dom_frame_per_unit { static constexpr bool value = false; };
template <> struct dom_frame_per_unit<FrameListArgs> { static constexpr bool value = true; };
VKD uint32_t dom_unit_frame(const FrameListArgs& fl, const RenderArgs& a, PathRng& rng) {
    const uint32_t f = rng.pixel / fl.fr.n_pix;
    dom_slot_rng(fl.fr, a, rng);
    return f;
}
template <class D> VKD void dom_accumulate(const D&, const RenderBuffers& buf, uint32_t pixel, float3 L) { accumulate_sample(buf, pixel, L); }
VKD void dom_accumulate(const ListArgs& ls, const RenderBuffers& buf, uint32_t pixel, float3 L) {
    accumulate_sample(buf, pixel, L);
    accumulate_square(ls.sq, pixel, L);
}
VKD void dom_accumulate(const FrameListArgs& fl, const RenderBuffers& buf, uint32_t pixel, float3 L) { dom_accumulate(fl.ls, buf, pixel, L); }
template <class D>
VKD bool mk_unit(const D&, const RenderArgs& a, uint32_t, uint32_t px0, uint32_t py0, uint32_t u, uint32_t& px, uint32_t& py, uint32_t& pixel) {
    px = px0 + (u & 7u);
    py = py0 + ((u >> 3) & 3u);
    if (!(px < a.width && py < a.height)) return false;
    pixel = py * a.width + px;
    return true;
}
VKD bool mk_unit(const ListArgs& ls, const RenderArgs& a, uint32_t tile, uint32_t, uint32_t, uint32_t u, uint32_t& px, uint32_t& py,
                 uint32_t& pixel) {
// ... 78 lines not shown
```

### vecchio_b200/csrc/vk_internal.h

```cpp
#pragma once
#include <cuda_runtime.h>
#include <stdint.h>

#include "../../include/vecchio_gpu.h"

#define VKD_DUP 0x08000000u
#define VKD_INDEX(r) ((r)&0x07FFFFFFu)
#define VKD_TYPE(r) ((r) >> 28)
#define VKD_T_EXIT 15u
#define VKD_STACK 96

struct DScene {
    const float4* wnodes;
    const float4* nodes;
    const float4* spheres;
    const uint32_t* sphere_mat;
    const float4* mspheres;
    const float4* rects;
    const float4* boxes;
    const float4* xforms;
    const float4* media;
    const float4* media_plan;
    const uint32_t* lights;
    const uint4* materials;
// ... 3 lines not shown
    const uint8_t* perlin_perm;
    const float4* flat_shade;
    const uint8_t* prim_cls;
    uint32_t cls_base[8];
    uint32_t root;
    uint32_t n_lights;
    uint32_t has_media;
    float4 light0_a, light0_b;
};
#define VKD_MAT_NEEDS_UV 0x80000000u

#define VKF_MAX_SEGS 12
#define VKF_MAX_OPS 24
#define VKF_MAX_RECTS 96
#define VKF_MAX_SPHERES 16
#define VKF_MAX_MEDIA 4
#define VKF_MAX_BVH 32
#define VKF_MAX_BOXES (VKF_MAX_RECTS / 6)
enum { VKF_OP_TRANSLATE = 0, VKF_OP_ROTX = 1, VKF_OP_ROTY = 2, VKF_OP_ROTZ = 3 };
struct FlatOp {
    uint32_t kind;
    float a, b, c;
};
struct FlatRect {
    float4 bounds;
    float k;
    uint32_t hit;
    uint32_t hitc;
    uint32_t _pad;
};

struct FlatSphere {
    float4 a;
    float4 b;
    float time1;
    uint32_t hit;
    uint32_t hitc;
    uint32_t _pad;
};
#define VKF_HITC(index, cls, inst) ((uint32_t)(index) | (((cls) == 0u ? 2u : (cls) == 1u ? 3u : (cls) == 2u ? 4u : ((inst) ? 6u : 5u)) << 8))
#define VKF_HIT_INDEX(id) ((id)&0xFFu)
struct FlatBox {
    float4 mn;
    float4 mx;
};
struct FlatMedium {
    float aff[12];
    float4 mn;
    float4 mx;
};
struct FlatHit {
    uint32_t prim;
    uint32_t inst;
    uint32_t face;
    uint32_t cls;
};
struct FlatSeg {
    uint8_t op0, op1;
    uint8_t rect0[6], rect1[6];
    uint8_t sph0, sph1;
    uint8_t msph0, msph1;
    uint8_t med0, med1;
    uint8_t bvh0, bvh1;
    uint8_t box0, box1;
};
struct FlatProgram {
    uint32_t n;
    uint32_t n_segs;
    uint32_t _pad[2];
    FlatSeg segs[VKF_MAX_SEGS];
    FlatOp ops[VKF_MAX_OPS];
    FlatRect rects[VKF_MAX_RECTS];
    FlatSphere spheres[VKF_MAX_SPHERES];
    FlatHit hits[VKF_MAX_RECTS + VKF_MAX_SPHERES + VKF_MAX_MEDIA];
    uint32_t n_bvh;
    uint32_t bvh[VKF_MAX_BVH];
    uint32_t seg_inst[VKF_MAX_SEGS];
    float seg_affine[VKF_MAX_SEGS][12];
    FlatBox boxes[VKF_MAX_BOXES];
    FlatMedium fmed[VKF_MAX_MEDIA];
    uint8_t seg_fm0[VKF_MAX_SEGS];
};

struct DCamera {
    float3 origin, lower_left_corner, horizontal, vertical, u, v;
    float lens_radius, time0, time1;
};

struct RenderArgs {
    uint32_t width, height;
    uint32_t spp_begin, spp_count;
    uint32_t max_depth;
    uint32_t seed_lo, seed_hi;
    float3 background;
    uint32_t flags;
    uint32_t tiles_x, tiles_y, n_chunks, chunk_spp;
};

struct OneFrame {};

struct FrameArgs {
    const DCamera* cams;
    uint32_t n_frames;
    uint32_t n_pix;
};

struct ListArgs {
    const uint32_t* list;
    uint32_t n;
    unsigned long long* sq;
};

struct FrameListArgs {
    FrameArgs fr;
    ListArgs ls;
};
#define VK_SQ_SCALE 4294967296.0f
#define VK_SQ_INV_SCALE (1.0 / 4294967296.0)
#define VK_SQ_CLAMP 255.0f
#define VK_ADAPTIVE_MAX_SPP 65536u

#define VK_ACC_SCALE 1073741824.0f
#define VK_ACC_INV_SCALE (1.0 / 1073741824.0)
struct RenderBuffers {
    unsigned long long* acc;
    double* accsq;
    unsigned long long* counters;
    unsigned long long* debug;
};
#define VK_DEBUG_CTAS 2048

enum { VKW_TERMINATE = 0, VKW_DIELECTRIC = 1, VKW_METAL = 2, VKW_DIFFUSE = 3, VKW_CLASSES = 4 };
struct WfState {
    float4* ray_o;
    float4* ray_d;
    float4* beta;
    uint4* unit;
    uint4* hit;
    uint32_t* queue;
    uint32_t* qcount;
    unsigned long long* unit_head;
    uint32_t n_slots;
    uint32_t n_pixels;
    unsigned long long n_units;
};

#define VK_DECLARE_LAUNCHERS(NS)                                                                                       \
    namespace NS {                                                                                                     \
    template <class D>                                                                                                 \
    cudaError_t launch_megakernel(const DScene& sc, const FlatProgram* flat, const DCamera& cam, const RenderArgs& a,  \
                                  const RenderBuffers& b, int grid, bool legacy, cudaStream_t st, const D& dom);       \
    template <class D>                                                                                                 \
    cudaError_t launch_megakernel_dyn(const DScene& sc, const DCamera& cam, const RenderArgs& a, const RenderBuffers& b, \
                                      unsigned long long* unit_head, int sm_count, cudaStream_t st, const D& dom);     \
    cudaError_t launch_intersect(const DScene& sc, const FlatProgram* flat, const vk_ray* rays, size_t n,              \
                                 const float* medium_xi, vk_hit* out, cudaStream_t st);                                \
    cudaError_t megakernel_occupancy(bool flat, bool media, bool legacy, int* blocks_per_sm, int* block_threads);      \
    cudaError_t launch_philox_kat(const uint32_t* ctr_key6, uint32_t* out4, cudaStream_t st);                          \
    cudaError_t launch_eval(const DScene& sc, vk_eval* recs, size_t n, uint32_t n_materials, uint32_t n_textures,      \
                            cudaStream_t st);                                                                          \
    cudaError_t launch_staged(const DScene& sc, const FlatProgram* flat, const DCamera& cam, const RenderArgs& a,      \
                              const RenderBuffers& b, unsigned long long* unit_head, int sm_count, cudaStream_t st);   \
    template <class D>                                                                                                 \
    cudaError_t launch_warpq(const DScene& sc, const FlatProgram* flat, const DCamera& cam, const RenderArgs& a,       \
                             const RenderBuffers& b, unsigned long long* unit_head, int sm_count, bool legacy,         \
                             cudaStream_t st, const D& dom);                                                           \
    size_t stepq_stack_words(uint32_t stack_need, bool inst, int sm_count, uint32_t* levels);                          \
    template <class D>                                                                                                 \
    cudaError_t launch_stepq(const DScene& sc, const DCamera& cam, const RenderArgs& a, const RenderBuffers& b,        \
                             unsigned long long* unit_head, uint32_t* gstack, uint32_t glevels, bool inst, int sm_count, \
                             bool legacy, cudaStream_t st, const D& dom);                                              \
    cudaError_t launch_wf_generate(const DCamera& cam, const RenderArgs& a, const WfState& w, cudaStream_t st);        \
    cudaError_t launch_wf_extend(const DScene& sc, const FlatProgram* flat, const RenderArgs& a, const WfState& w,     \
                                 const RenderBuffers& b, uint32_t set, cudaStream_t st);                               \
    cudaError_t launch_wf_shade(const DScene& sc, const DCamera& cam, const RenderArgs& a, const WfState& w,           \
                                const RenderBuffers& b, uint32_t set, cudaStream_t st);                                \
    }
VK_DECLARE_LAUNCHERS(vkfast)
VK_DECLARE_LAUNCHERS(vkstrict)
VK_DECLARE_LAUNCHERS(vkfast_l0)
namespace vkfast_simple {
cudaError_t launch_staged(const DScene& sc, const FlatProgram* flat, const DCamera& cam, const RenderArgs& a, const RenderBuffers& b,
                          unsigned long long* unit_head, int sm_count, cudaStream_t st);
template <class D>
cudaError_t launch_warpq(const DScene& sc, const FlatProgram* flat, const DCamera& cam, const RenderArgs& a, const RenderBuffers& b,
                         unsigned long long* unit_head, int sm_count, bool legacy, cudaStream_t st, const D& dom);
}
```

### vecchio_b200/csrc/vk_relayout.cu

```cuda
#include <cstdio>
#include <cstdlib>

#include "vk_relayout.h"

using namespace vkhost;

extern "C" {

int vk_scene_check(const vk_scene_desc* d, vk_scene_info* info, char* err, size_t err_len) {
    auto report = [&](int code, const std::string& msg) {
        if (err && err_len) std::snprintf(err, err_len, "%s", msg.c_str());
        return code;
    };
    if (!d) return report(VK_ERR_INVALID, "null scene");
    Validator v;
    v.d = d;
    if (!v.run()) return report(v.code, v.err);
    Relayout R;
    if (const char* why = R.run(d)) return report(VK_ERR_UNSUPPORTED, why);
    if (info) {
        info->flat_entries = R.flat.n;
        info->flat_segments = R.flat.n ? R.flat.n_segs : 0;
        info->flat_subtrees = R.flat.n ? R.flat.n_bvh : 0;
        info->simple = R.simple ? 1u : 0u;
        info->wide_nodes = R.n_wide;
        info->stack_need = R.stack_need;
        info->wide_levels_world = R.levels_world;
        info->wide_levels_instance = R.levels_sub;
        info->dynamic_megakernel = d->n_nodes >= 65536u ? 1u : 0u;
        info->flat_boxes = 0;
        for (uint32_t s = 0; R.flat.n && s < R.flat.n_segs; ++s) info->flat_boxes += R.flat.segs[s].box1 - R.flat.segs[s].box0;
        info->flat_direct = 0;
        for (size_t h = 0; 2 * h + 1 < R.flat_shade.size(); ++h) info->flat_direct += __float_as_uint_host(R.flat_shade[2 * h].w) & 1u;
    }
    if (err && err_len) err[0] = 0;
    return VK_OK;
}

}
```

### vecchio_b200/csrc/vk_relayout.h

```cpp
#pragma once
#include <cstdint>
#include <cstdlib>
#include <cstring>
#include <string>
#include <utility>
#include <vector>

#include "vk_internal.h"

namespace vkhost {

inline uint32_t __float_as_uint_host(float f) {
    uint32_t u;
    std::memcpy(&u, &f, 4);
    return u;
}
inline float __uint_as_float_host(uint32_t u) {
    float f;
    std::memcpy(&f, &u, 4);
    return f;
}
struct Validator {
    const vk_scene_desc* d;
    std::string err;
// ... 383 lines not shown
                const uint32_t hz = g.rects[3][b.at[0]].first.hit, hy = g.rects[4][b.at[1]].first.hit, hx = g.rects[5][b.at[2]].first.hit;
                FlatBox& fb = P->boxes[n_boxes++];
                fb.mn = make_float4(b.mn[0], b.mn[1], b.mn[2], __uint_as_float_host(hz));
                fb.mx = make_float4(b.mx[0], b.mx[1], b.mx[2], __uint_as_float_host(hy | (hx << 16)));
            }
            o.box1 = (uint8_t)n_boxes;
            if (n_sph + g.sph.size() + g.msph.size() > VKF_MAX_SPHERES) return false;
            o.sph0 = (uint8_t)n_sph;
            for (auto& e : g.sph) {
                e.first.hit = n_hits;
                P->hits[n_hits++] = e.second;
                P->spheres[n_sph++] = e.first;
            }
            o.sph1 = o.msph0 = (uint8_t)n_sph;
            for (auto& e : g.msph) {
                e.first.hit = n_hits;
                P->hits[n_hits++] = e.second;
                P->spheres[n_sph++] = e.first;
            }
            o.msph1 = (uint8_t)n_sph;
            if (n_med + g.med.size() > VKF_MAX_MEDIA) return false;
            o.med0 = (uint8_t)n_hits;
            P->seg_fm0[s] = (uint8_t)n_med;
            for (const FlatHit& h : g.med) {
                FlatMedium& fm = P->fmed[n_med];
                fm = FlatMedium{};
                const vk_medium& md = d->media[VK_REF_INDEX(h.prim & ~VKD_DUP)];
                std::vector<FlatOp> ops;
                const vk_ref leaf = chain_ops(d, md.boundary, ops);
                compose_flat_ops(ops.data(), ops.size(), fm.aff);
                if (VK_REF_TYPE(leaf) == VK_T_BOX) {
                    const vk_box& b = d->boxes[VK_REF_INDEX(leaf)];
                    fm.mn = make_float4(b.box_min[0], b.box_min[1], b.box_min[2], md.neg_inv_density);
                    fm.mx = make_float4(b.box_max[0], b.box_max[1], b.box_max[2], __uint_as_float_host(1u | (ops.empty() ? 0u : 2u)));
                }
                P->hits[n_hits++] = h;
                ++n_med;
            }
            o.med1 = (uint8_t)n_hits;
            if (n_bvh + g.bvh.size() > VKF_MAX_BVH) return false;
            o.bvh0 = (uint8_t)n_bvh;
            for (uint32_t r : g.bvh) P->bvh[n_bvh++] = r;
            o.bvh1 = (uint8_t)n_bvh;
            P->seg_inst[s] = g.inst;
            compose_flat_ops(g.ops.data(), g.ops.size(), P->seg_affine[s]);
        }
        P->n_bvh = n_bvh;
        for (uint32_t h = 0; h < n_hits; ++h) {
            const vk_ref pr = P->hits[h].prim & ~VKD_DUP;
            const uint32_t i = VK_REF_INDEX(pr);
            uint32_t mat = 0;
            switch (VK_REF_TYPE(pr)) {
            case VK_T_SPHERE: mat = d->sphere_mat[i]; break;
            case VK_T_MSPHERE: mat = d->mspheres[i].mat; break;
            case VK_T_RECT: mat = d->rects[i].mat; break;
            case VK_T_BOX: mat = d->boxes[i].mat; break;
            case VK_T_MEDIUM: mat = d->media[i].mat; break;
            default: return false;
            }
            const uint32_t t = d->materials[mat].type;
            P->hits[h].cls = t == VK_M_DIFFUSE_LIGHT ? 0u : t == VK_M_DIELECTRIC ? 1u : t == VK_M_METAL ? 2u : 3u;
        }
        static_assert(VKF_MAX_RECTS + VKF_MAX_SPHERES + VKF_MAX_MEDIA <= 256, "class-tagged ids keep the entry in 8 bits");
        auto tagged = [&](uint32_t h) { return VKF_HITC(h, P->hits[h].cls, P->hits[h].inst); };
        for (uint32_t i = 0; i < n_rects; ++i) P->rects[i].hitc = tagged(P->rects[i].hit);
        for (uint32_t i = 0; i < n_sph; ++i) P->spheres[i].hitc = tagged(P->spheres[i].hit);
        for (uint32_t i = 0; i < n_boxes; ++i) {
            const uint32_t hz = __float_as_uint_host(P->boxes[i].mn.w), hyx = __float_as_uint_host(P->boxes[i].mx.w);
            P->boxes[i].mn.w = __uint_as_float_host(tagged(hz));
            P->boxes[i].mx.w = __uint_as_float_host(tagged(hyx & 0xFFFFu) | (tagged(hyx >> 16) << 16));
        }
        P->n_segs = (uint32_t)segs.size();
        P->n = n_hits + n_bvh;
        return P->n > 0;
    }
};

struct Relayout {
    std::vector<vk_node> nodes;
    std::vector<float4> wnodes;
    FlatProgram flat{};
    uint32_t levels_world = 0, levels_sub = 0, n_wide = 0, stack_need = 0;
    bool simple = false, has_specdiffuse = false;
    std::vector<float4> flat_shade;
    std::vector<float4> media_plan;
    const char* run(const vk_scene_desc* d) {
        nodes.assign(d->nodes, d->nodes + d->n_nodes);
        for (uint32_t i = 0; i < d->n_nodes; ++i)
            if (nodes[i].left == nodes[i].right) {
                vk_ref end = nodes[i].left;
                while (VK_REF_TYPE(end) == VK_T_XFORM) end = d->xforms[VK_REF_INDEX(end)].child;
                nodes[i].right = VK_REF_TYPE(end) == VK_T_MEDIUM ? (nodes[i].left | VKD_DUP) : VK_REF_NONE;
            }
        wnodes.assign((size_t)d->n_nodes * 8, make_float4(0, 0, 0, 0));
        {
            struct Slot {
                vk_ref ref;
                float mn[3], mx[3];
            };
            std::vector<uint8_t> built(d->n_nodes, 0);
            std::vector<uint32_t> todo, level(d->n_nodes, 0);
            levels_world = levels_sub = 0;
            bool in_sub = false;
            auto want = [&](vk_ref r, uint32_t lvl) {
                if (VK_REF_TYPE(r) == VK_T_NODE && !built[VK_REF_INDEX(r)]) {
                    built[VK_REF_INDEX(r)] = 1;
                    level[VK_REF_INDEX(r)] = lvl;
                    todo.push_back(VK_REF_INDEX(r));
                    uint32_t& top = in_sub ? levels_sub : levels_world;
                    if (lvl + 1 > top) top = lvl + 1;
                }
            };
            auto child_slot = [&](vk_ref r, const vk_node& parent) {
                const vk_node& b = VK_REF_TYPE(r) == VK_T_NODE ? d->nodes[VK_REF_INDEX(r)] : parent;
                Slot s{r, {b.bb_min[0], b.bb_min[1], b.bb_min[2]}, {b.bb_max[0], b.bb_max[1], b.bb_max[2]}};
                return s;
            };
            auto area = [](const Slot& s) {
                const float x = s.mx[0] - s.mn[0], y = s.mx[1] - s.mn[1], z = s.mx[2] - s.mn[2];
                return x * y + y * z + z * x;
            };
            for (int pass = 0; pass < 2; ++pass) {
            in_sub = pass == 1;
            if (pass == 0) want(d->root, 0);
            else
                for (uint32_t i = 0; i < d->n_xforms; ++i) want(d->xforms[i].child, 0);
            while (!todo.empty()) {
                const uint32_t ni = todo.back();
                todo.pop_back();
                Slot slots[6];
                size_t n_slots = 0;
                auto add_children = [&](uint32_t n) {
                    if (nodes[n].left != VK_REF_NONE) slots[n_slots++] = child_slot(nodes[n].left, d->nodes[n]);
                    if (nodes[n].right != VK_REF_NONE) slots[n_slots++] = child_slot(nodes[n].right, d->nodes[n]);
                };
                add_children(ni);
                while (n_slots < 4) {
                    int best = -1;
                    for (size_t k = 0; k < n_slots; ++k)
                        if (VK_REF_TYPE(slots[k].ref) == VK_T_NODE) {
                            const uint32_t n = VK_REF_INDEX(slots[k].ref);
                            const size_t kids = (nodes[n].left != VK_REF_NONE) + (nodes[n].right != VK_REF_NONE);
                            if (n_slots - 1 + kids > 4) continue;
                            if (best < 0 || area(slots[k]) > area(slots[best])) best = (int)k;
                        }
                    if (best < 0) break;
                    const uint32_t n = VK_REF_INDEX(slots[best].ref);
                    for (size_t k = (size_t)best; k + 1 < n_slots; ++k) slots[k] = slots[k + 1];
                    --n_slots;
                    add_children(n);
                }
                ++n_wide;
                float4* q = &wnodes[(size_t)ni * 8];
                float* f = reinterpret_cast<float*>(q);
                for (size_t k = 0; k < 4; ++k) {
                    const bool have = k < n_slots;
                    for (int ax = 0; ax < 3; ++ax) {
                        f[(2 * ax) * 4 + k] = have ? slots[k].mn[ax] : 0.f;
                        f[(2 * ax + 1) * 4 + k] = have ? slots[k].mx[ax] : 0.f;
                    }
                    f[6 * 4 + k] = __uint_as_float_host(have ? slots[k].ref : VK_REF_NONE);
                    if (have) want(slots[k].ref, level[ni] + 1);
                }
            }
            }
            if (3 * levels_world + 1 + 3 * levels_sub + 2 > VKD_STACK)
                return "BVH deeper than the traversal stack";
        }
        stack_need = 3 * levels_world + 1 + 3 * levels_sub + 2;
        FlatBuilder fb;
        fb.d = d;
        if (!fb.build(&flat, false)) {
            const bool heterogeneous = d->n_media > 0 || d->n_xforms > 0;
            const char* hy = std::getenv("VECCHIO_HYBRID");
            if (!(heterogeneous && !(hy && hy[0] == '0') && fb.build(&flat, true) && flat.n_bvh > 0)) flat = FlatProgram{};
        }
        media_plan.assign(4 * (size_t)d->n_media, make_float4(0, 0, 0, 0));
        for (uint32_t i = 0; i < d->n_media; ++i) {
            std::vector<FlatOp> ops;
            const vk_ref leaf = chain_ops(d, d->media[i].boundary, ops);
            float m[12];
            compose_flat_ops(ops.data(), ops.size(), m);
            for (int r = 0; r < 3; ++r) media_plan[4 * i + r] = make_float4(m[3 * r], m[3 * r + 1], m[3 * r + 2], m[9 + r]);
            media_plan[4 * i + 3] = make_float4(__uint_as_float_host(leaf), __uint_as_float_host(ops.empty() ? 0u : 1u), 0.f, 0.f);
        }
        flat_shade.clear();
        if (flat.n && flat.n_bvh == 0) {
            Validator tv;
            tv.d = d;
            flat_shade.assign(2 * (size_t)flat.n, make_float4(0, 0, 0, 0));
            for (uint32_t h = 0; h < flat.n; ++h) {
                const FlatHit& fh = flat.hits[h];
                const vk_ref pr = fh.prim & ~VKD_DUP;
                const uint32_t i = VK_REF_INDEX(pr);
                uint32_t a2, flip, mat;
                flat_shade[2 * h + 1] = make_float4(0.f, __uint_as_float_host(pr),
                                                    __uint_as_float_host((fh.inst ? (0x80000000u | VKD_INDEX(fh.inst)) : 0u) | (fh.face << 28)), 0.f);
                if (VK_REF_TYPE(pr) == VK_T_RECT) {
                    a2 = (d->rects[i].axes >> 4) & 3u;
                    flip = (d->rects[i].axes & VK_RECT_FLIP) ? 1u : 0u;
                    mat = d->rects[i].mat;
                } else if (VK_REF_TYPE(pr) == VK_T_BOX) {
                    a2 = fh.face < 2 ? 2u : (fh.face < 4 ? 1u : 0u);
                    flip = fh.face & 1u;
                    mat = d->boxes[i].mat;
                } else
                    continue;
                const vk_material& m = d->materials[mat];
                const bool reads_uv = m.type == VK_M_SPECDIFFUSE || (m.type != VK_M_DIELECTRIC && tv.tex_has_image(m.tex, 0));
                const bool reads_front = m.type == VK_M_DIELECTRIC || m.type == VK_M_DIFFUSE_LIGHT || m.type == VK_M_SPECDIFFUSE;
                float n[3] = {a2 == 0 ? 1.f : 0.f, a2 == 1 ? 1.f : 0.f, a2 == 2 ? 1.f : 0.f};
                bool ok = !reads_uv;
                if (fh.inst) {
                    std::vector<vk_xform> chain;
                    vk_ref r = fh.inst;
                    while (VK_REF_TYPE(r) == VK_T_XFORM) {
                        chain.push_back(d->xforms[VK_REF_INDEX(r)]);
                        r = chain.back().child;
                    }
                    ok = ok && !reads_front && !chain.empty() && chain.front().kind == VK_X_TRANSLATE;
                    for (size_t l = chain.size(); l-- > 0 && ok;) {
                        const vk_xform& x = chain[l];
                        const float sn = x.a, cs = x.b, v0 = n[0], v1 = n[1], v2 = n[2];
                        if (x.kind == VK_X_ROTATE_Y) { n[0] = cs * v0 + sn * v2; n[2] = -sn * v0 + cs * v2; }
                        else if (x.kind == VK_X_ROTATE_X) { n[1] = cs * v1 - sn * v2; n[2] = sn * v1 + cs * v2; }
                        else if (x.kind == VK_X_ROTATE_Z) { n[0] = cs * v0 - sn * v1; n[1] = sn * v0 + cs * v1; }
                        else if (x.kind == VK_X_FLIP) ok = false;
                    }
                }
                if (!ok) continue;
                flat_shade[2 * h] = make_float4(n[0], n[1], n[2], __uint_as_float_host(1u | (flip << 1)));
                flat_shade[2 * h + 1].x = __uint_as_float_host(mat);
            }
        }
        has_specdiffuse = false;
        for (uint32_t i = 0; i < d->n_materials; ++i) has_specdiffuse |= d->materials[i].type == VK_M_SPECDIFFUSE;
        simple = d->n_mspheres == 0 && d->n_lights == 1 && VK_REF_TYPE(d->lights[0]) == VK_T_RECT &&
                 !(d->rects[VK_REF_INDEX(d->lights[0])].axes & VK_RECT_FLIP);
        for (uint32_t i = 0; i < d->n_textures && simple; ++i) simple = d->textures[i].type == VK_TEX_SOLID;
        for (uint32_t i = 0; i < d->n_materials && simple; ++i)
            simple = d->materials[i].type == VK_M_LAMBERTIAN || d->materials[i].type == VK_M_DIELECTRIC ||
                     d->materials[i].type == VK_M_DIFFUSE_LIGHT || d->materials[i].type == VK_M_ISOTROPIC;
        return nullptr;
    }
};


}
```

### vecchio_b200/csrc/vk_warpq.cu

```cuda
#include "vk_warpq.cuh"

namespace VK_NS {

template <bool MEDIA, bool LEGACY, class W, int K, bool HYBRID, class D>
VKD void warpq_flat_body(const DScene& sc, const FlatProgram* flat, const DCamera& cam, const RenderArgs& a, const RenderBuffers& buf,
                         unsigned long long* unit_head, const D& dom) {
    extern __shared__ __align__(16) unsigned char vkq_raw[];
    const uint32_t lane = threadIdx.x & 31u, below = (1u << lane) - 1u;
    W& S = reinterpret_cast<W*>(vkq_raw)[threadIdx.x >> 5];
    const WqCtx<W> C = wq_ctx(dom, cam, a, S, unit_head, lane);
    uint32_t n_rays = 0, n_drop = 0, n_prims = 0;
    TraceCounters tc = {0u, 0u};
    constexpr uint32_t EXT_CAP = 32u * K;
    const uint32_t miss_cls = wq_black_miss(a) ? (uint32_t)VKQ_END : (uint32_t)VKQ_EMIT;
    wq_init(S, lane);
#pragma unroll 1
    for (;;) {
        uint32_t q, n_q, tail_q, head;
        wq_selfcheck(S, buf, lane, 0u);
        if (!wq_pick(S, wq_counts(S), EXT_CAP, q, n_q, tail_q)) break;
        const uint32_t n = wq_pop(S, q, n_q, tail_q, q == VKQ_EXT ? EXT_CAP : 32u, lane, head);
        if (q != VKQ_EXT) {
            wq_shade_batch<LEGACY, !HYBRID>(sc, C, dom, buf, q, n, head, n_drop);
            continue;
        }
        wq_converge();
        float3 o[K], d[K];
        float tm[K], best_t[K];
        bool live[K];
        uint32_t best_hit[K], slot[K];
        MediumXi xi[K];
#pragma unroll
        for (int k = 0; k < K; ++k) {
            const uint32_t e = lane + 32u * k;
            live[k] = e < n;
            slot[k] = S.ring[VKQ_EXT][(head + (live[k] ? e : 0u)) & W::RMASK];
            const float4 ro = S.ro[slot[k]], rd = S.rd[slot[k]];
            o[k] = f3(ro);
            d[k] = f3(rd);
            tm[k] = ro.w;
            xi[k].table = nullptr;
            xi[k].depth = __float_as_uint(rd.w);
            xi[k].rng.key = make_uint2(a.seed_lo, a.seed_hi);
            xi[k].rng.pixel = MEDIA ? S.px[slot[k]] : 0u;
            xi[k].rng.sample = MEDIA ? __float_as_uint(S.bt[slot[k]].w) : 0u;
            if (MEDIA) dom_slot_rng(dom, a, xi[k].rng);
        }
        TraceHit sub[K];
        trace_flat_k<K, MEDIA, HYBRID>(sc, *flat, o, d, tm, live, 0.001f, xi, best_t, best_hit, sub, &tc);
#pragma unroll
        for (int k = 0; k < K; ++k) {
            uint32_t cls = VKQ_NONE;
            if (live[k]) {
                ++n_rays;
                n_prims += flat->n;
                uint32_t prim = VK_REF_NONE, hi = 0u;
                cls = miss_cls;
                if (HYBRID && best_hit[k] == 0xFFFFFFFEu) {
                    prim = sub[k].prim;
                    hi = (sub[k].inst ? (0x80000000u | VKD_INDEX(sub[k].inst)) : 0u) | (sub[k].face << 28);
                    cls = wq_class_of(sc, prim, sub[k].inst);
                } else if (best_hit[k] != 0xFFFFFFFFu) {
                    cls = best_hit[k] >> 8;
                    best_hit[k] = VKF_HIT_INDEX(best_hit[k]);
                    prim = 1u;
                    if (HYBRID) {
                        const FlatHit& fh = flat->hits[best_hit[k]];
                        prim = fh.prim & ~VKD_DUP;
                        hi = (fh.inst ? (0x80000000u | VKD_INDEX(fh.inst)) : 0u) | (fh.face << 28);
                    }
                }
                S.hp[slot[k]] = make_uint4(__float_as_uint(best_t[k]), prim, hi, best_hit[k]);
            }
            if (k == 0 || n > 32u * k) wq_push(S, cls, slot[k], lane, below);
        }
    }
    wq_flush_counters(buf, lane, n_rays, n_drop, tc.nodes, n_prims + tc.prims);
}

#ifndef VKQ_BVH_IDLE
#define VKQ_BVH_IDLE 8u
#endif
#ifndef VKQ_NODE_STEPS
#define VKQ_NODE_STEPS 4
#endif
template <bool MEDIA, bool LEGACY, class W, class D>
VKD void warpq_bvh_body(const DScene& sc, const DCamera& cam, const RenderArgs& a, const RenderBuffers& buf, unsigned long long* unit_head,
                        const D& dom) {
    extern __shared__ __align__(16) unsigned char vkq_raw[];
    const uint32_t lane = threadIdx.x & 31u, below = (1u << lane) - 1u;
    W& S = reinterpret_cast<W*>(vkq_raw)[threadIdx.x >> 5];
    const WqCtx<W> C = wq_ctx(dom, cam, a, S, unit_head, lane);
    uint32_t n_rays = 0, n_drop = 0;
    TraceCounters tc = {0u, 0u};
    const uint32_t miss_cls = wq_black_miss(a) ? (uint32_t)VKQ_END : (uint32_t)VKQ_EMIT;
    wq_init(S, lane);

    Trav T;
    T.ref = VKD_DONE;
    T.sp = 0;
    T.enter = false;
    T.cur_inst = 0;
    T.co = T.cd = T.cinv = f3(0.0f, 0.0f, 0.0f);
    T.best.t = 0.0f;
    T.best.prim = VK_REF_NONE;
    T.best.inst = 0;
    T.best.face = 0;
    float3 o = f3(0.0f, 0.0f, 0.0f), d = o;
    float tm = 0.0f;
    uint32_t cur = 0xFFFFFFFFu;
    MediumXi xi;
    xi.table = nullptr;
    xi.depth = 0;
    xi.rng.key = make_uint2(a.seed_lo, a.seed_hi);
    xi.rng.pixel = 0;
    xi.rng.sample = 0;
#pragma unroll 1
    for (;;) {
        const bool done_lane = T.ref == VKD_DONE;
        const uint32_t m_done = __ballot_sync(0xFFFFFFFFu, done_lane);
        if ((uint32_t)__popc(m_done) >= VKQ_BVH_IDLE) {
            const bool fin = done_lane && cur != 0xFFFFFFFFu;
            if (__ballot_sync(0xFFFFFFFFu, fin) != 0u) {
                uint32_t cls = VKQ_NONE, slot = 0u;
                if (fin) {
                    slot = cur;
                    cur = 0xFFFFFFFFu;
                    S.hp[slot] = make_uint4(__float_as_uint(T.best.t), T.best.prim,
                                            (T.best.inst ? (0x80000000u | VKD_INDEX(T.best.inst)) : 0u) | (T.best.face << 28), 0u);
                    cls = T.best.prim == VK_REF_NONE ? miss_cls : wq_class_of(sc, T.best.prim, T.best.inst);
                }
                wq_push(S, cls, slot, lane, below);
            }
            wq_selfcheck(S, buf, lane, (uint32_t)__popc(__ballot_sync(0xFFFFFFFFu, cur != 0xFFFFFFFFu)));
            const WqCounts cnt = wq_counts(S);
            const uint32_t n_ext = __reduce_max_sync(0xFFFFFFFFu, cnt.c01.x);
            if (n_ext != 0u) {
                uint32_t head;
                const uint32_t take = wq_pop(S, VKQ_EXT, n_ext, cnt.c01.y, (uint32_t)__popc(m_done), lane, head);
                const uint32_t rank = (uint32_t)__popc(m_done & below);
                if (done_lane && rank < take) {
                    cur = S.ring[VKQ_EXT][(head + rank) & W::RMASK];
                    const float4 ro = S.ro[cur], rd = S.rd[cur];
                    o = f3(ro);
                    d = f3(rd);
                    tm = ro.w;
                    xi.depth = __float_as_uint(rd.w);
                    if (MEDIA) {
                        xi.rng.pixel = S.px[cur];
                        xi.rng.sample = __float_as_uint(S.bt[cur].w);
                        dom_slot_rng(dom, a, xi.rng);
                    }
                    trav_init(T, sc, o, d, CUDART_INF_F);
                    ++n_rays;
                }
            }
            const uint32_t m_act = __ballot_sync(0xFFFFFFFFu, T.ref != VKD_DONE);
            if (32u - (uint32_t)__popc(m_act) >= VKQ_BVH_IDLE) {
                uint32_t q, n_q, tail_q, head;
                if (wq_pick(S, wq_counts(S), 0u, q, n_q, tail_q)) {
                    const uint32_t n = wq_pop(S, q, n_q, tail_q, 32u, lane, head);
                    wq_shade_batch<LEGACY, false>(sc, C, dom, buf, q, n, head, n_drop);
                    continue;
                }
                if (m_act == 0u) break;
            }
        }
        wq_converge();
#pragma unroll 1
        for (int k = 0; k < VKQ_NODE_STEPS && trav_at_node(T); ++k) trav_node_step(T, sc, 0.001f, tc);
        if (T.ref != VKD_DONE && !trav_at_node(T)) trav_prim_step<MEDIA>(T, sc, o, d, tm, 0.001f, xi, tc);
    }
    wq_flush_counters(buf, lane, n_rays, n_drop, tc.nodes, tc.prims);
}

using WqFlat = WqWarp<VKQ_N_FLAT, VKQ_RN_FLAT>;
using WqMedia = WqWarp<VKQ_N_MEDIA, VKQ_RN_MEDIA>;
using WqBvh = WqWarp<VKQ_N_BVH, VKQ_RN_BVH>;
using WqHyb = WqWarp<VKQ_N_HYB, VKQ_RN_HYB>;
static_assert(VKQ_WARPS <= 15, "one named barrier per warp of the CTA");

template <bool MEDIA, bool LEGACY, class D>
__global__ void __launch_bounds__(32 * VKQ_WARPS, VKQ_MINB_BVH) k_warpq(const DScene sc, const DCamera cam, const RenderArgs a, const RenderBuffers buf,
                                                                    unsigned long long* unit_head, const __grid_constant__ D dom) {
    warpq_bvh_body<MEDIA, LEGACY, WqBvh>(sc, cam, a, buf, unit_head, dom);
}
template <bool LEGACY, class D>
__global__ void __launch_bounds__(32 * VKQ_WARPS, VKQ_MINB_FLAT) k_warpq_flat(const DScene sc, const __grid_constant__ FlatProgram flat, const DCamera cam,
                                                                          const RenderArgs a, const RenderBuffers buf, unsigned long long* unit_head,
                                                                          const __grid_constant__ D dom) {
    warpq_flat_body<false, LEGACY, WqFlat, VKQ_K_FLAT, false>(sc, &flat, cam, a, buf, unit_head, dom);
}
template <bool LEGACY, class D>
__global__ void __launch_bounds__(32 * VKQ_WARPS, VKQ_MINB_MEDIA) k_warpq_flat_media(const DScene sc, const __grid_constant__ FlatProgram flat,
                                                                                 const DCamera cam, const RenderArgs a, const RenderBuffers buf,
                                                                                 unsigned long long* unit_head, const __grid_constant__ D dom) {
    warpq_flat_body<true, LEGACY, WqMedia, VKQ_K_MEDIA, false>(sc, &flat, cam, a, buf, unit_head, dom);
}
#if !VK_SIMPLE
template <bool MEDIA, bool LEGACY, class D>
__global__ void __launch_bounds__(32 * VKQ_WARPS, VKQ_MINB_HYB) k_warpq_hybrid(const DScene sc, const __grid_constant__ FlatProgram flat, const DCamera cam,
                                                                            const RenderArgs a, const RenderBuffers buf, unsigned long long* unit_head,
                                                                            const __grid_constant__ D dom) {
    warpq_flat_body<MEDIA, LEGACY, WqHyb, 1, true>(sc, &flat, cam, a, buf, unit_head, dom);
}
#endif

template <class D>
cudaError_t launch_warpq(const DScene& sc, const FlatProgram* flat, const DCamera& cam, const RenderArgs& a, const RenderBuffers& b,
                         unsigned long long* unit_head, int sm_count, bool legacy, cudaStream_t st, const D& dom) {
    int bps = 0;
    cudaError_t e;
    const bool media = sc.has_media != 0u;
#define VKQ_LAUNCH_FLAT(KERNEL, WARP)                                                                                  \
    {                                                                                                                  \
        const size_t smem = VKQ_WARPS * sizeof(WARP);                                                                  \
        if ((e = warpq_prepare(KERNEL, smem, &bps)) != cudaSuccess) return e;                                          \
        KERNEL<<<sm_count * (bps < 1 ? 1 : bps), 32 * VKQ_WARPS, smem, st>>>(sc, *flat, cam, a, b, unit_head, dom);    \
    }
#define VKQ_LAUNCH_BVH(KERNEL)                                                                                         \
    {                                                                                                                  \
        const size_t smem = VKQ_WARPS * sizeof(WqBvh);                                                                 \
        if ((e = warpq_prepare(KERNEL, smem, &bps)) != cudaSuccess) return e;                                          \
        KERNEL<<<sm_count * (bps < 1 ? 1 : bps), 32 * VKQ_WARPS, smem, st>>>(sc, cam, a, b, unit_head, dom);           \
    }
#if VK_SIMPLE
    (void)legacy;
    if (media) VKQ_LAUNCH_FLAT((k_warpq_flat_media<false, D>), WqMedia) else VKQ_LAUNCH_FLAT((k_warpq_flat<false, D>), WqFlat)
#else
#define VKQ_LAUNCH_HYB(M, G) VKQ_LAUNCH_FLAT((k_warpq_hybrid<M, G, D>), WqHyb)
    if (flat && flat->n && flat->n_bvh) {
        if (media) { if (legacy) VKQ_LAUNCH_HYB(true, true) else VKQ_LAUNCH_HYB(true, false) }
        else { if (legacy) VKQ_LAUNCH_HYB(false, true) else VKQ_LAUNCH_HYB(false, false) }
    } else if (flat && flat->n) {
        if (media) { if (legacy) VKQ_LAUNCH_FLAT((k_warpq_flat_media<true, D>), WqMedia) else VKQ_LAUNCH_FLAT((k_warpq_flat_media<false, D>), WqMedia) }
        else { if (legacy) VKQ_LAUNCH_FLAT((k_warpq_flat<true, D>), WqFlat) else VKQ_LAUNCH_FLAT((k_warpq_flat<false, D>), WqFlat) }
    } else {
        if (media) { if (legacy) VKQ_LAUNCH_BVH((k_warpq<true, true, D>)) else VKQ_LAUNCH_BVH((k_warpq<true, false, D>)) }
        else { if (legacy) VKQ_LAUNCH_BVH((k_warpq<false, true, D>)) else VKQ_LAUNCH_BVH((k_warpq<false, false, D>)) }
    }
#undef VKQ_LAUNCH_HYB
#endif
#undef VKQ_LAUNCH_FLAT
#undef VKQ_LAUNCH_BVH
    return cudaGetLastError();
}
#define VKQ_INSTANTIATE(D)                                                                                             \
    template cudaError_t launch_warpq(const DScene&, const FlatProgram*, const DCamera&, const RenderArgs&, const RenderBuffers&, \
                                      unsigned long long*, int, bool, cudaStream_t, const D&);
VKQ_INSTANTIATE(OneFrame)
VKQ_INSTANTIATE(FrameArgs)
VKQ_INSTANTIATE(ListArgs)
VKQ_INSTANTIATE(FrameListArgs)
#undef VKQ_INSTANTIATE

}
```

### vecchio_b200/csrc/vk_warpq.cuh

```cuda
#pragma once
#include "vk_device.cuh"

namespace VK_NS {

#ifndef VKQ_WARPS
#define VKQ_WARPS 4
#endif
#ifndef VKQ_N_FLAT
#define VKQ_N_FLAT 176
#endif
#ifndef VKQ_RN_FLAT
#define VKQ_RN_FLAT 256
#endif
#ifndef VKQ_K_FLAT
#define VKQ_K_FLAT 2
#endif
#ifndef VKQ_MINB_FLAT
#define VKQ_MINB_FLAT 4
#endif
#ifndef VKQ_N_MEDIA
#define VKQ_N_MEDIA 144
#endif
#ifndef VKQ_RN_MEDIA
#define VKQ_RN_MEDIA 256
// ... 196 lines not shown
        if (C.lane == 0) {
            S.cur_x = cx + take;
            S.left = left - take;
        }
        __syncwarp();
        served += take;
    }
    if (got) {
        PathRng rng;
        rng.pixel = y * C.a.width + x;
        rng.sample = C.a.spp_begin + s;
        rng.key = make_uint2(C.a.seed_lo, C.a.seed_hi);
        float3 o, d;
        float time;
        const uint32_t p = wq_camera_ray(C, dom, x, y, rng, o, d, time);
        S.ro[slot] = make_float4(o.x, o.y, o.z, time);
        S.rd[slot] = make_float4(d.x, d.y, d.z, __uint_as_float(1u));
        S.bt[slot] = make_float4(1.0f, 1.0f, 1.0f, __uint_as_float(rng.sample));
        S.px[slot] = p;
        S.mark_new(slot);
    }
    return got;
}

VKD bool wq_black_miss(const RenderArgs& a) {
    return !(a.flags & VK_FLAG_SKY_BACKGROUND) && a.background.x == 0.0f && a.background.y == 0.0f && a.background.z == 0.0f;
}
VKD uint32_t wq_class_of(const DScene& sc, uint32_t prim, uint32_t inst) {
    uint32_t mat;
    const uint32_t i = VKD_INDEX(prim);
    switch (VKD_TYPE(prim)) {
    case VK_T_SPHERE: mat = __ldg(&sc.sphere_mat[i]); break;
    case VK_T_MSPHERE: mat = __float_as_uint(__ldg(&sc.mspheres[3 * i + 2]).y); break;
    case VK_T_RECT: mat = __float_as_uint(__ldg(&sc.rects[2 * i + 1]).z); break;
    case VK_T_BOX: mat = __float_as_uint(__ldg(&sc.boxes[2 * i]).w); break;
    default: mat = __float_as_uint(__ldg(&sc.media[i]).z); break;
    }
    const uint32_t t = __ldg(&sc.materials[mat]).x;
    return t == VK_M_DIFFUSE_LIGHT ? VKQ_EMIT : t == VK_M_DIELECTRIC ? VKQ_DIEL : t == VK_M_METAL ? VKQ_METAL : (inst ? VKQ_DIFFI : VKQ_DIFF);
}

struct WqCounts {
    uint4 c01, c23, c45, c67;
};
template <class W>
VKD WqCounts wq_counts(const W& S) {
    WqCounts c;
    c.c01 = *reinterpret_cast<const uint4*>(&S.ct[0]);
    c.c23 = *reinterpret_cast<const uint4*>(&S.ct[2]);
    c.c45 = *reinterpret_cast<const uint4*>(&S.ct[4]);
    c.c67 = *reinterpret_cast<const uint4*>(&S.ct[6]);
    return c;
}
template <class W>
VKD bool wq_pick(const W& S, const WqCounts& c, uint32_t ext_cap, uint32_t& q, uint32_t& n_q, uint32_t& tail_q) {
    const uint32_t w = (ext_cap ? ext_cap : 32u) * 8u;
    uint32_t key = ext_cap ? c.c01.x * 256u + VKQ_EXT : 0u;
    key = max(key, c.c23.x * w + VKQ_EMIT);
    key = max(key, c.c45.z * w + VKQ_DIFF);
    key = max(key, c.c67.x * w + VKQ_DIFFI);
    key = max(key, c.c23.z * w + VKQ_DIEL);
    key = max(key, c.c45.x * w + VKQ_METAL);
    key = max(key, c.c01.z * w + VKQ_END);
    key = __reduce_max_sync(0xFFFFFFFFu, key);
    q = key & 7u;
    const uint2 e = S.ct[q];
    n_q = e.x;
    tail_q = e.y;
    return (key >> 3) != 0u;
}
template <class W>
VKD uint32_t wq_pop(W& S, uint32_t q, uint32_t n_q, uint32_t tail_q, uint32_t cap, uint32_t lane, uint32_t& head) {
    const uint32_t n = min(n_q, cap);
    head = tail_q - n_q;
    __syncwarp();
    if (lane == 0) S.ct[q].x = n_q - n;
    __syncwarp();
    return n;
}

#ifndef VKQ_FAST_RESOLVE
#define VKQ_FAST_RESOLVE 1
#endif
template <bool LEGACY, bool FLAT, class W, class D>
VKD void wq_shade_batch(const DScene& sc, const WqCtx<W>& C, const D& dom, const RenderBuffers& buf, uint32_t q, uint32_t n, uint32_t head, uint32_t& n_drop) {
    W& S = C.S;
    const RenderArgs& a = C.a;
    const uint32_t lane = C.lane;
    const bool act = lane < n;
    const uint32_t slot = S.ring[q][(head + (act ? lane : 0u)) & W::RMASK];
    bool alive = false, ended = false;
    if (q != VKQ_END) {
        if (act) {
            const float4 ro = S.ro[slot], rd = S.rd[slot], bt = S.bt[slot];
            const uint4 hp = S.hp[slot];
            float3 o = f3(ro), d = f3(rd), beta = f3(bt), L = f3(0.0f, 0.0f, 0.0f);
            float time = ro.w;
            uint32_t depth = __float_as_uint(rd.w);
            const uint32_t pixel = S.px[slot], prim = hp.y;
            bool valid = true;
            if (prim == VK_REF_NONE) {
                L = beta * miss_color(a, d);
            } else {
                PathRng rng;
                rng.pixel = pixel;
                rng.sample = __float_as_uint(bt.w);
                rng.key = make_uint2(a.seed_lo, a.seed_hi);
                dom_slot_rng(dom, a, rng);
                HitRecD rec;
                bool direct = false;
                uint32_t leaf = prim, hi = hp.z;
                if (FLAT) {
                    const float4 fs1 = __ldg(&sc.flat_shade[2u * hp.w + 1u]);
                    leaf = __float_as_uint(fs1.y);
                    hi = __float_as_uint(fs1.z);
#if VKQ_FAST_RESOLVE && !VK_STRICT
                    const float4 fs = __ldg(&sc.flat_shade[2u * hp.w]);
                    const uint32_t fl = __float_as_uint(fs.w);
                    if (fl & 1u) {
                        direct = true;
                        const float3 nw = f3(fs);
                        const bool toward = dot3(d, nw) < 0.0f;
                        rec.t = __uint_as_float(hp.x);
                        rec.p = at(o, d, rec.t);
                        rec.normal = toward ? nw : -nw;
                        rec.front = (toward ? 1u : 0u) ^ ((fl >> 1) & 1u);
                        rec.u = 0.0f;
                        rec.v = 0.0f;
                        rec.mat = __float_as_uint(fs1.x);
                        rec.m = __ldg(&sc.materials[rec.mat]);
                    }
#endif
                }
                if (!direct) {
                    TraceHit h;
                    h.t = __uint_as_float(hp.x);
                    h.prim = leaf;
                    h.inst = (hi & 0x80000000u) ? (((uint32_t)VK_T_XFORM << 28) | (hi & 0x07FFFFFFu)) : 0u;
                    h.face = (hi >> 28) & 7u;
                    resolve_hit(sc, h, o, d, time, false, rec);
                }
                alive = LEGACY ? shade_legacy(sc, rec, rng, depth, o, d, time, beta, L, valid)
                               : shade(sc, rec, rng, depth, o, d, time, beta, L, valid);
                if (alive && ++depth > a.max_depth) alive = false;
                if (alive && !(finite3(d) && finite3(o))) {
                    valid = false;
                    alive = false;
                }
            }
            if (alive) {
                S.ro[slot] = make_float4(o.x, o.y, o.z, time);
                S.rd[slot] = make_float4(d.x, d.y, d.z, __uint_as_float(depth));
                S.bt[slot] = make_float4(beta.x, beta.y, beta.z, bt.w);
                S.mark_new(slot);
            } else {
                if (valid && finite3(L)) dom_accumulate(dom, buf, pixel, L);
                else ++n_drop;
                ended = true;
            }
        }
    } else {
        ended = act;
    }
    const uint32_t m_end = __ballot_sync(0xFFFFFFFFu, ended);
    bool to_end = false;
    if (q == VKQ_END || (uint32_t)__popc(m_end) >= VKQ_REGEN_MIN) alive = wq_regen(C, dom, ended, slot) || alive;
    else to_end = ended;
    const uint32_t m_ext = __ballot_sync(0xFFFFFFFFu, alive), m_q = __ballot_sync(0xFFFFFFFFu, to_end);
    const uint2 c_ext = S.ct[VKQ_EXT], c_end = S.ct[VKQ_END];
    if (alive) S.ring[VKQ_EXT][(c_ext.y + __popc(m_ext & C.below)) & W::RMASK] = (uint8_t)slot;
    if (to_end) S.ring[VKQ_END][(c_end.y + __popc(m_q & C.below)) & W::RMASK] = (uint8_t)slot;
    __syncwarp();
    if (lane == 0) {
        S.ct[VKQ_EXT] = make_uint2(c_ext.x + (uint32_t)__popc(m_ext), c_ext.y + (uint32_t)__popc(m_ext));
        if (m_q) S.ct[VKQ_END] = make_uint2(c_end.x + (uint32_t)__popc(m_q), c_end.y + (uint32_t)__popc(m_q));
    }
    __syncwarp();
}

#ifndef VKQ_SELFCHECK
#define VKQ_SELFCHECK 0
#endif
template <class W>
VKD void wq_selfcheck(const W& S, const RenderBuffers& buf, uint32_t lane, uint32_t in_flight) {
#if VKQ_SELFCHECK
    uint32_t seen[8] = {0, 0, 0, 0, 0, 0, 0, 0};
    uint32_t bad = 0, total = 0;
    for (uint32_t q = 0; q < W::NQ; ++q) {
        const uint2 c = S.ct[q];
        total += c.x;
        if (c.x > W::N) ++bad;
        for (uint32_t i0 = 0; i0 < c.x; i0 += 32u) {
            const uint32_t i = i0 + lane;
            const bool have = i < c.x;
            const uint32_t slot = have ? S.ring[q][(c.y - c.x + i) & W::RMASK] : 0u;
            if (have && slot >= W::N) ++bad;
            const uint32_t same = __match_any_sync(0xFFFFFFFFu, have ? slot : 0x10000u + lane);
            if (have && __popc(same) != 1) ++bad;
#pragma unroll
            for (uint32_t w = 0; w < 8; ++w) {
                const uint32_t mine = (have && (slot >> 5) == w) ? (1u << (slot & 31u)) : 0u;
                const uint32_t all = __reduce_or_sync(0xFFFFFFFFu, mine);
                if (mine & seen[w]) ++bad;
                seen[w] |= all;
            }
        }
    }
    if (total + in_flight > W::N) ++bad;
    if (bad) atomicAdd(&buf.counters[5], (unsigned long long)bad);
#else
    (void)S, (void)buf, (void)lane, (void)in_flight;
#endif
}

template <class W>
VKD void wq_init(W& S, uint32_t lane) {
    if (lane < W::NQ + (W::NQ & 1u)) S.ct[lane] = make_uint2(0u, 0u);
    for (uint32_t i = lane; i < W::N; i += 32u) S.ring[VKQ_END][i] = (uint8_t)i;
    if (lane == 0) {
        S.left = 0u;
        S.exhausted = 0u;
        S.cur_s = 0u;
        S.cur_y = 0u;
        S.cur_x = 0u;
    }
    __syncwarp();
    if (lane == 0) S.ct[VKQ_END] = make_uint2(W::N, W::N);
    __syncwarp();
}
VKD void wq_flush_counters(const RenderBuffers& buf, uint32_t lane, uint32_t n_rays, uint32_t n_drop, uint32_t n_nodes, uint32_t n_prims) {
    unsigned long long w_rays = n_rays, w_drop = n_drop, w_nodes = n_nodes, w_prims = n_prims;
#pragma unroll
    for (int off = 16; off > 0; off >>= 1) {
        w_rays += __shfl_xor_sync(0xFFFFFFFFu, w_rays, off);
        w_drop += __shfl_xor_sync(0xFFFFFFFFu, w_drop, off);
        w_nodes += __shfl_xor_sync(0xFFFFFFFFu, w_nodes, off);
        w_prims += __shfl_xor_sync(0xFFFFFFFFu, w_prims, off);
    }
    if (lane == 0) {
        atomicAdd(&buf.counters[3], w_nodes);
        atomicAdd(&buf.counters[4], w_prims);
        atomicAdd(&buf.counters[0], w_rays);
        if (w_drop) atomicAdd(&buf.counters[1], w_drop);
    }
}

// ... 22 lines not shown
```

Before: 11590.

## Add compile-time static flat-scene kernel and per-material-class shading bodies

Factors the per-primitive flat intersection loops into reusable helpers. It adds a statically specialised warp-queue kernel for recognised simple scene shapes (such as Cornell), where the primitive list is fixed at compile time. It also lets each queue batch be shaded by a material-class-specific body (emitter, dielectric, diffuse) instead of the generic shade switch. The aim is to cut divergence, branches and constant loads in the simple-scene path, at the cost of larger code and extra kernel instantiations. A scene-shape field is added to the scene info, and an env var disables the static path.

```diff
diff --git a/include/vecchio_gpu.h b/include/vecchio_gpu.h
--- a/include/vecchio_gpu.h
+++ b/include/vecchio_gpu.h
@@ -241,6 +241,7 @@
     uint32_t dynamic_megakernel;
     uint32_t flat_boxes;
     uint32_t flat_direct;
+    uint32_t flat_shape;
 } vk_scene_info;
 int vk_scene_check(const vk_scene_desc* scene, vk_scene_info* info, char* err, size_t err_len);
 
diff --git a/profiles/make_sass_counts.py b/profiles/make_sass_counts.py
--- /dev/null
+++ b/profiles/make_sass_counts.py
@@ -0,0 +1,66 @@
+#!/usr/bin/env python
+import collections
+import re
+import subprocess
+import sys
+
+CUOBJDUMP = "/usr/local/cuda/bin/cuobjdump"
+KERNELS = [("k_warpq_flat", r"k_warpq_flatILb0E8OneFrame"), ("k_warpq_flat_static<Cornell>", r"k_warpq_flat_static.*8OneFrame")]
+ROWS = ["BRA", "BSSY", "BSYNC", "NOP", "LDCU.U8", "LDCU", "LDC", "MOV", "UMOV", "IMAD.MOV", "ISETP", "UISETP", "FFMA", "FMUL", "FADD",
+        "FSETP", "FSEL", "FMNMX", "MUFU", "LDS", "STS", "SHFL", "VOTE"]
+
+
+def kernels(obj):
+    text = subprocess.run([CUOBJDUMP, "-sass", obj], capture_output=True, text=True, check=True).stdout
+    out, cur = {}, None
+    for line in text.splitlines():
+        m = re.match(r"\s*Function : (\S+)", line)
+        if m:
+            cur = m.group(1)
+            out[cur] = []
+            continue
+        m = re.match(r"\s*/\*[0-9a-f]{4,}\*/\s+(.*?);", line)
+        if m and cur:
+            ins = re.sub(r"^@!?U?P\w+\s+", "", m.group(1).strip())
+            out[cur].append(ins.split()[0])
+    return out
+
+
+def classify(op):
+    if op.startswith("LDCU.U8"):
+        return "LDCU.U8"
+    if op.startswith("IMAD.MOV"):
+        return "IMAD.MOV"
+    base = op.split(".")[0]
+    return base if base in ROWS else "other"
+
+
+def counts(obj, pat):
+    ks = kernels(obj)
+    hit = [k for k in ks if re.search(pat, k)]
+    if not hit:
+        return None
+    c = collections.Counter(classify(op) for op in ks[hit[0]])
+    c["total"] = len(ks[hit[0]])
+    return c
+
+
+def main():
+    before, after = sys.argv[1], sys.argv[2]
+    cols = [("before: " + KERNELS[0][0], counts(before, KERNELS[0][1]))]
+    cols += [("after: " + name, counts(after, pat)) for name, pat in KERNELS]
+    cols = [(n, c) for n, c in cols if c is not None]
+    print("# Static SASS instruction counts of the Cornell warp-queue kernel (sm_100a, `cuobjdump -sass`)\n")
+    print("Made by `profiles/make_sass_counts.py` from `vecchio_b200/csrc/vk_warpq_simple.o` of the parent commit (before) and of this")
+    print("change (after), `OneFrame` instances.  Static counts: each instruction of the kernel's code once, not how often it runs.")
+    print("`k_warpq_flat` is the generic kernel (`VECCHIO_NO_STATIC_FLAT=1`, and every simple scene without a compiled shape);")
+    print("after the change both kernels shade each batch with its queue's class body.\n")
+    print("| class | " + " | ".join(n for n, _ in cols) + " |")
+    print("|---|" + "---|" * len(cols))
+    for r in ROWS + ["other", "total"]:
+        print(f"| `{r}` | " + " | ".join(str(c.get(r, 0)) for _, c in cols) + " |")
+    print("| code KB | " + " | ".join(f"{c['total'] * 16 / 1024:.1f}" for _, c in cols) + " |")
+
+
+if __name__ == "__main__":
+    main()
diff --git a/vecchio_b200/_abi.py b/vecchio_b200/_abi.py
--- a/vecchio_b200/_abi.py
+++ b/vecchio_b200/_abi.py
@@ -107,7 +107,7 @@
 
 class vk_scene_info(C.Structure):
     _fields_ = [(n, C.c_uint32) for n in ("flat_entries", "flat_segments", "flat_subtrees", "simple", "wide_nodes", "wide_levels_world",
-                                          "wide_levels_instance", "stack_need", "dynamic_megakernel", "flat_boxes", "flat_direct")]
+                                          "wide_levels_instance", "stack_need", "dynamic_megakernel", "flat_boxes", "flat_direct", "flat_shape")]
 
 
 class vk_ray(C.Structure):
diff --git a/vecchio_b200/csrc/vk_api.cu b/vecchio_b200/csrc/vk_api.cu
--- a/vecchio_b200/csrc/vk_api.cu
+++ b/vecchio_b200/csrc/vk_api.cu
@@ -40,6 +40,7 @@
     bool has_specdiffuse = false;
     bool simple_scene = false;
     bool one_rect_light = false;
+    uint32_t flat_shape = VKF_SHAPE_NONE;
     unsigned long long* debug = nullptr;
     unsigned long long* counters = nullptr;
     float* partial = nullptr;
@@ -449,6 +450,7 @@
     c->wnodes_bytes = wnodes.size() * sizeof(float4);
     c->has_specdiffuse = R.has_specdiffuse;
     c->simple_scene = R.simple;
+    c->flat_shape = R.flat_shape;
     c->one_rect_light = d->n_lights == 1 && VK_REF_TYPE(d->lights[0]) == VK_T_RECT && !(d->rects[VK_REF_INDEX(d->lights[0])].axes & VK_RECT_FLIP);
     c->stack_need = R.stack_need;
     c->levels_sub = R.levels_sub;
@@ -697,10 +699,11 @@
             CU(c, cudaMemsetAsync(c->counters + 5, 0, sizeof(unsigned long long), c->stream));
             const FlatProgram* sflat = flat;
             const bool simple = !strict && !legacy && sflat && sflat->n_bvh == 0 && c->simple_scene && !std::getenv("VECCHIO_NO_SIMPLE");
-            CU(c, strict   ? vkstrict::launch_warpq(c->scene, sflat, dc, a, b, c->counters + 2, c->sm_count, legacy, c->stream, dom)
-                  : simple ? vkfast_simple::launch_warpq(c->scene, sflat, dc, a, b, c->counters + 2, c->sm_count, legacy, c->stream, dom)
-                  : l0     ? vkfast_l0::launch_warpq(c->scene, sflat, dc, a, b, c->counters + 2, c->sm_count, legacy, c->stream, dom)
-                           : vkfast::launch_warpq(c->scene, sflat, dc, a, b, c->counters + 2, c->sm_count, legacy, c->stream, dom));
+            const uint32_t shape = std::getenv("VECCHIO_NO_STATIC_FLAT") ? (uint32_t)VKF_SHAPE_NONE : c->flat_shape;
+            CU(c, strict   ? vkstrict::launch_warpq(c->scene, sflat, VKF_SHAPE_NONE, dc, a, b, c->counters + 2, c->sm_count, legacy, c->stream, dom)
+                  : simple ? vkfast_simple::launch_warpq(c->scene, sflat, shape, dc, a, b, c->counters + 2, c->sm_count, legacy, c->stream, dom)
+                  : l0     ? vkfast_l0::launch_warpq(c->scene, sflat, VKF_SHAPE_NONE, dc, a, b, c->counters + 2, c->sm_count, legacy, c->stream, dom)
+                           : vkfast::launch_warpq(c->scene, sflat, VKF_SHAPE_NONE, dc, a, b, c->counters + 2, c->sm_count, legacy, c->stream, dom));
             *launches += 1;
         } else if (variant == VK_VARIANT_WAVEFRONT) {
             uint32_t n = 0;
diff --git a/vecchio_b200/csrc/vk_device.cuh b/vecchio_b200/csrc/vk_device.cuh
--- a/vecchio_b200/csrc/vk_device.cuh
+++ b/vecchio_b200/csrc/vk_device.cuh
@@ -591,30 +591,32 @@
 }
 #if !VK_STRICT
 template <int K>
+VKD void flat_box_k(const FlatBox& bx, const float3 (&co)[K], const float3 (&ci)[K], float tmin, float (&best_t)[K], uint32_t (&best_hit)[K]) {
+    const float4 mn = bx.mn, mx = bx.mx;
+    const uint32_t hz = __float_as_uint(mn.w), hy = __float_as_uint(mx.w) & 0xFFFFu, hx = __float_as_uint(mx.w) >> 16;
+#pragma unroll
+    for (int q = 0; q < K; ++q) {
+        const float x0 = (mn.x - co[q].x) * ci[q].x, x1 = (mx.x - co[q].x) * ci[q].x;
+        const float y0 = (mn.y - co[q].y) * ci[q].y, y1 = (mx.y - co[q].y) * ci[q].y;
+        const float z0 = (mn.z - co[q].z) * ci[q].z, z1 = (mx.z - co[q].z) * ci[q].z;
+        const float nx = fminf(x0, x1), ny = fminf(y0, y1), nz = fminf(z0, z1);
+        const float fx = fmaxf(x0, x1), fy = fmaxf(y0, y1), fz = fmaxf(z0, z1);
+        const float t_near = fmaxf(fmaxf(nx, ny), nz), t_far = fminf(fminf(fx, fy), fz);
+        const bool enter = t_near >= tmin;
+        const float t = enter ? t_near : t_far;
+        const bool hit = (t_near <= t_far) & (t >= tmin) & (t < best_t[q]);
+        const bool on_z = (enter ? nz : fz) == t, on_y = (enter ? ny : fy) == t;
+        const float at_max = on_z ? z1 : (on_y ? y1 : x1);
+        const uint32_t id = (on_z ? hz : (on_y ? hy : hx)) + (at_max == t ? 0u : 1u);
+        best_t[q] = hit ? t : best_t[q];
+        best_hit[q] = hit ? id : best_hit[q];
+    }
+}
+template <int K>
 VKD void flat_boxes_k(const FlatProgram& P, uint32_t i0, uint32_t i1, const float3 (&co)[K], const float3 (&ci)[K], float tmin,
                       float (&best_t)[K], uint32_t (&best_hit)[K]) {
 #pragma unroll 1
-    for (uint32_t i = i0; i < i1; ++i) {
-        const float4 mn = P.boxes[i].mn, mx = P.boxes[i].mx;
-        const uint32_t hz = __float_as_uint(mn.w), hy = __float_as_uint(mx.w) & 0xFFFFu, hx = __float_as_uint(mx.w) >> 16;
-#pragma unroll
-        for (int q = 0; q < K; ++q) {
-            const float x0 = (mn.x - co[q].x) * ci[q].x, x1 = (mx.x - co[q].x) * ci[q].x;
-            const float y0 = (mn.y - co[q].y) * ci[q].y, y1 = (mx.y - co[q].y) * ci[q].y;
-            const float z0 = (mn.z - co[q].z) * ci[q].z, z1 = (mx.z - co[q].z) * ci[q].z;
-            const float nx = fminf(x0, x1), ny = fminf(y0, y1), nz = fminf(z0, z1);
-            const float fx = fmaxf(x0, x1), fy = fmaxf(y0, y1), fz = fmaxf(z0, z1);
-            const float t_near = fmaxf(fmaxf(nx, ny), nz), t_far = fminf(fminf(fx, fy), fz);
-            const bool enter = t_near >= tmin;
-            const float t = enter ? t_near : t_far;
-            const bool hit = (t_near <= t_far) & (t >= tmin) & (t < best_t[q]);
-            const bool on_z = (enter ? nz : fz) == t, on_y = (enter ? ny : fy) == t;
-            const float at_max = on_z ? z1 : (on_y ? y1 : x1);
-            const uint32_t id = (on_z ? hz : (on_y ? hy : hx)) + (at_max == t ? 0u : 1u);
-            best_t[q] = hit ? t : best_t[q];
-            best_hit[q] = hit ? id : best_hit[q];
-        }
-    }
+    for (uint32_t i = i0; i < i1; ++i) flat_box_k<K>(P.boxes[i], co, ci, tmin, best_t, best_hit);
 }
 #endif
 template <bool MEDIA>
@@ -729,36 +731,39 @@
 }
 
 template <int K, int AX, bool BOX_SIDE>
+VKD void flat_rect_k(const FlatRect& r, const float3 (&co)[K], const float3 (&cd)[K], const float3 (&ci)[K], float tmin, float (&best_t)[K],
+                     uint32_t (&best_hit)[K]) {
+    const float4 bd = r.bounds;
+    const float k = r.k;
+    const uint32_t id = r.hitc;
+#pragma unroll
+    for (int q = 0; q < K; ++q) {
+        float tt, a, b;
+        if (AX == 0) {
+            tt = VKF_PLANE_T(k, co[q].z, cd[q].z, ci[q].z);
+            a = co[q].x + tt * cd[q].x;
+            b = co[q].y + tt * cd[q].y;
+        } else if (AX == 1) {
+            tt = VKF_PLANE_T(k, co[q].y, cd[q].y, ci[q].y);
+            a = co[q].x + tt * cd[q].x;
+            b = co[q].z + tt * cd[q].z;
+        } else {
+            tt = VKF_PLANE_T(k, co[q].x, cd[q].x, ci[q].x);
+            a = co[q].y + tt * cd[q].y;
+            b = co[q].z + tt * cd[q].z;
+        }
+        bool miss = (a < bd.x) | (a > bd.y) | (b < bd.z) | (b > bd.w) | (tt < tmin);
+        miss = miss | (tt > best_t[q]);
+        if (BOX_SIDE) miss = miss | !(tt < best_t[q]);
+        best_t[q] = miss ? best_t[q] : tt;
+        best_hit[q] = miss ? best_hit[q] : id;
+    }
+}
+template <int K, int AX, bool BOX_SIDE>
 VKD void flat_rects_k(const FlatProgram& P, uint32_t i0, uint32_t i1, const float3 (&co)[K], const float3 (&cd)[K], const float3 (&ci)[K],
                       float tmin, float (&best_t)[K], uint32_t (&best_hit)[K]) {
 #pragma unroll 1
-    for (uint32_t i = i0; i < i1; ++i) {
-        const float4 bd = P.rects[i].bounds;
-        const float k = P.rects[i].k;
-        const uint32_t id = P.rects[i].hitc;
-#pragma unroll
-        for (int q = 0; q < K; ++q) {
-            float tt, a, b;
-            if (AX == 0) {
-                tt = VKF_PLANE_T(k, co[q].z, cd[q].z, ci[q].z);
-                a = co[q].x + tt * cd[q].x;
-                b = co[q].y + tt * cd[q].y;
-            } else if (AX == 1) {
-                tt = VKF_PLANE_T(k, co[q].y, cd[q].y, ci[q].y);
-                a = co[q].x + tt * cd[q].x;
-                b = co[q].z + tt * cd[q].z;
-            } else {
-                tt = VKF_PLANE_T(k, co[q].x, cd[q].x, ci[q].x);
-                a = co[q].y + tt * cd[q].y;
-                b = co[q].z + tt * cd[q].z;
-            }
-            bool miss = (a < bd.x) | (a > bd.y) | (b < bd.z) | (b > bd.w) | (tt < tmin);
-            miss = miss | (tt > best_t[q]);
-            if (BOX_SIDE) miss = miss | !(tt < best_t[q]);
-            best_t[q] = miss ? best_t[q] : tt;
-            best_hit[q] = miss ? best_hit[q] : id;
-        }
-    }
+    for (uint32_t i = i0; i < i1; ++i) flat_rect_k<K, AX, BOX_SIDE>(P.rects[i], co, cd, ci, tmin, best_t, best_hit);
 }
 #if !VK_STRICT
 #ifndef VKF_INLINE_MEDIA
@@ -798,6 +803,32 @@
     return true;
 }
 #endif
+template <int K>
+VKD void flat_sphere_k(const FlatSphere& s, const float3 (&co)[K], const float3 (&cd)[K], float tmin, float (&best_t)[K], uint32_t (&best_hit)[K]) {
+    const float4 sp = s.a;
+    const uint32_t id = s.hitc;
+#pragma unroll
+    for (int q = 0; q < K; ++q) {
+        float tt;
+        if (sphere_t(f3(sp), sp.w, co[q], cd[q], tmin, best_t[q], tt)) {
+            best_t[q] = tt;
+            best_hit[q] = id;
+        }
+    }
+}
+template <int K>
+VKD void flat_affine_k(const float* m, const float3 (&wo)[K], const float3 (&wd)[K], float3 (&co)[K], float3 (&cd)[K]) {
+    const float r00 = m[0], r01 = m[1], r02 = m[2], r10 = m[3], r11 = m[4], r12 = m[5], r20 = m[6], r21 = m[7], r22 = m[8];
+    const float t0 = m[9], t1 = m[10], t2 = m[11];
+#pragma unroll
+    for (int q = 0; q < K; ++q) {
+        const float3 o = wo[q], d = wd[q];
+        co[q] = f3(fmaf(r00, o.x, fmaf(r01, o.y, fmaf(r02, o.z, t0))), fmaf(r10, o.x, fmaf(r11, o.y, fmaf(r12, o.z, t1))),
+                   fmaf(r20, o.x, fmaf(r21, o.y, fmaf(r22, o.z, t2))));
+        cd[q] = f3(fmaf(r00, d.x, fmaf(r01, d.y, r02 * d.z)), fmaf(r10, d.x, fmaf(r11, d.y, r12 * d.z)),
+                   fmaf(r20, d.x, fmaf(r21, d.y, r22 * d.z)));
+    }
+}
 template <int K, bool MEDIA, bool HYBRID>
 VKD void flat_segment_k(const DScene& sc, const FlatProgram& P, const FlatSeg& g, uint32_t s, const float3 (&o)[K], const float3 (&d)[K],
                         const float3 (&co)[K], const float3 (&cd)[K], const float (&time)[K], const bool (&live)[K], float tmin,
@@ -816,18 +847,7 @@
     flat_boxes_k<K>(P, g.box0, g.box1, co, ci, tmin, best_t, best_hit);
 #endif
 #pragma unroll 1
-    for (uint32_t i = g.sph0; i < g.sph1; ++i) {
-        const float4 sp = P.spheres[i].a;
-        const uint32_t id = P.spheres[i].hitc;
-#pragma unroll
-        for (int q = 0; q < K; ++q) {
-            float tt;
-            if (sphere_t(f3(sp), sp.w, co[q], cd[q], tmin, best_t[q], tt)) {
-                best_t[q] = tt;
-                best_hit[q] = id;
-            }
-        }
-    }
+    for (uint32_t i = g.sph0; i < g.sph1; ++i) flat_sphere_k<K>(P.spheres[i], co, cd, tmin, best_t, best_hit);
 #if !VK_SIMPLE
 #pragma unroll 1
     for (uint32_t i = g.msph0; i < g.msph1; ++i) {
@@ -917,19 +937,7 @@
     for (uint32_t s = 1; s < n_segs; ++s) {
         const FlatSeg& g = P.segs[s];
         float3 co[K], cd[K];
-        {
-            const float* m = P.seg_affine[s];
-            const float r00 = m[0], r01 = m[1], r02 = m[2], r10 = m[3], r11 = m[4], r12 = m[5], r20 = m[6], r21 = m[7], r22 = m[8];
-            const float t0 = m[9], t1 = m[10], t2 = m[11];
-#pragma unroll
-            for (int q = 0; q < K; ++q) {
-                const float3 wo = o[q], wd = d[q];
-                co[q] = f3(fmaf(r00, wo.x, fmaf(r01, wo.y, fmaf(r02, wo.z, t0))), fmaf(r10, wo.x, fmaf(r11, wo.y, fmaf(r12, wo.z, t1))),
-                           fmaf(r20, wo.x, fmaf(r21, wo.y, fmaf(r22, wo.z, t2))));
-                cd[q] = f3(fmaf(r00, wd.x, fmaf(r01, wd.y, r02 * wd.z)), fmaf(r10, wd.x, fmaf(r11, wd.y, r12 * wd.z)),
-                           fmaf(r20, wd.x, fmaf(r21, wd.y, r22 * wd.z)));
-            }
-        }
+        flat_affine_k<K>(P.seg_affine[s], o, d, co, cd);
         flat_segment_k<K, MEDIA, HYBRID>(sc, P, g, s, o, d, co, cd, time, live, tmin, xi, best_t, best_hit, sub, tc);
     }
     return;
@@ -960,24 +968,54 @@
             }
         }
 #else
-        if (g.op1 != g.op0) {
-            const float* m = P.seg_affine[s];
-            const float r00 = m[0], r01 = m[1], r02 = m[2], r10 = m[3], r11 = m[4], r12 = m[5], r20 = m[6], r21 = m[7], r22 = m[8];
-            const float t0 = m[9], t1 = m[10], t2 = m[11];
-#pragma unroll
-            for (int q = 0; q < K; ++q) {
-                const float3 wo = co[q], wd = cd[q];
-                co[q] = f3(fmaf(r00, wo.x, fmaf(r01, wo.y, fmaf(r02, wo.z, t0))), fmaf(r10, wo.x, fmaf(r11, wo.y, fmaf(r12, wo.z, t1))),
-                           fmaf(r20, wo.x, fmaf(r21, wo.y, fmaf(r22, wo.z, t2))));
-                cd[q] = f3(fmaf(r00, wd.x, fmaf(r01, wd.y, r02 * wd.z)), fmaf(r10, wd.x, fmaf(r11, wd.y, r12 * wd.z)),
-                           fmaf(r20, wd.x, fmaf(r21, wd.y, r22 * wd.z)));
-            }
-        }
+        if (g.op1 != g.op0) flat_affine_k<K>(P.seg_affine[s], o, d, co, cd);
 #endif
         flat_segment_k<K, MEDIA, HYBRID>(sc, P, g, s, o, d, co, cd, time, live, tmin, xi, best_t, best_hit, sub, tc);
     }
     }
 }
+
+#if !VK_STRICT
+template <class G, int K>
+VKD void flat_segment_static(const FlatProgram& P, const float3 (&co)[K], const float3 (&cd)[K], float tmin, float (&best_t)[K],
+                             uint32_t (&best_hit)[K]) {
+    float3 ci[K];
+#pragma unroll
+    for (int q = 0; q < K; ++q) ci[q] = rcp3(cd[q]);
+#pragma unroll
+    for (int i = G::x0; i < G::x1; ++i) flat_rect_k<K, 0, false>(P.rects[i], co, cd, ci, tmin, best_t, best_hit);
+#pragma unroll
+    for (int i = G::y0; i < G::y1; ++i) flat_rect_k<K, 1, false>(P.rects[i], co, cd, ci, tmin, best_t, best_hit);
+#pragma unroll
+    for (int i = G::z0; i < G::z1; ++i) flat_rect_k<K, 2, false>(P.rects[i], co, cd, ci, tmin, best_t, best_hit);
+#pragma unroll
+    for (int i = G::b0; i < G::b1; ++i) flat_box_k<K>(P.boxes[i], co, ci, tmin, best_t, best_hit);
+#pragma unroll
+    for (int i = G::s0; i < G::s1; ++i) flat_sphere_k<K>(P.spheres[i], co, cd, tmin, best_t, best_hit);
+}
+template <int K, int S, class G, class... Rest>
+VKD void flat_segments_static(const FlatProgram& P, const float3 (&o)[K], const float3 (&d)[K], float tmin, float (&best_t)[K],
+                              uint32_t (&best_hit)[K]) {
+    if constexpr (S == 0) {
+        flat_segment_static<G, K>(P, o, d, tmin, best_t, best_hit);
+    } else {
+        float3 co[K], cd[K];
+        flat_affine_k<K>(P.seg_affine[S], o, d, co, cd);
+        flat_segment_static<G, K>(P, co, cd, tmin, best_t, best_hit);
+    }
+    if constexpr (sizeof...(Rest) > 0) flat_segments_static<K, S + 1, Rest...>(P, o, d, tmin, best_t, best_hit);
+}
+template <int K, class... Seg>
+VKD void trace_flat_static(const FlatProgram& P, FlatShape<Seg...>, const float3 (&o)[K], const float3 (&d)[K], float tmin, float (&best_t)[K],
+                           uint32_t (&best_hit)[K]) {
+#pragma unroll
+    for (int q = 0; q < K; ++q) {
+        best_t[q] = CUDART_INF_F;
+        best_hit[q] = 0xFFFFFFFFu;
+    }
+    flat_segments_static<K, 0, Seg...>(P, o, d, tmin, best_t, best_hit);
+}
+#endif
 
 struct HitRecD {
     float3 p, normal;
@@ -1409,40 +1447,94 @@
     VKD uint4 block0() const { return r; }
     VKD uint32_t spec() const { return s; }
 };
+VKD bool shade_emitter(const DScene& sc, const HitRecD& rec, const uint4& m, const float3& beta, float3& L) {
+    float3 emitted = f3(0.0f, 0.0f, 0.0f);
+    if (rec.front) emitted = tex_value(sc, m.y, rec.u, rec.v, rec.p);
+    L = L + beta * emitted;
+    return false;
+}
+VKD bool shade_dielectric(const HitRecD& rec, const uint4& m, const uint4& r, float3& o, float3& d) {
+    const float ref_idx = __uint_as_float(m.z);
+    const float etai_over_etat = rec.front ? 1.0f / ref_idx : ref_idx;
+    const float3 unit_direction = unit_vector(d);
+    const float cos_theta = fminf(dot3(-unit_direction, rec.normal), 1.0f);
+    const float sin_theta = sqrtf(1.0f - cos_theta * cos_theta);
+    float3 nd;
+    if (etai_over_etat * sin_theta > 1.0f) nd = reflect(unit_direction, rec.normal);
+    else if (u01(r.x) < schlick(cos_theta, etai_over_etat)) nd = reflect(unit_direction, rec.normal);
+    else nd = refract(unit_direction, rec.normal, etai_over_etat);
+    o = rec.p;
+    d = nd;
+    return true;
+}
+VKD bool shade_diffuse(const DScene& sc, const HitRecD& rec, const uint4& m, uint32_t spdf_type, const uint4& r, float3& o, float3& d,
+                       float3& beta, bool& valid) {
+    const float3 attenuation = tex_value(sc, m.y, rec.u, rec.v, rec.p);
+#if VK_STRICT
+    const Onb uvw = onb_from_w(rec.normal);
+    const float3 onb_w = uvw.w;
+#else
+    const float3 onb_w = unit_vector(rec.normal);
+#endif
+    float3 nd;
+    if (u01(r.x) < 0.5f) {
+#if VK_SIMPLE || VK_LIGHT0
+        nd = rect_random(sc.light0_a, sc.light0_b.x, __float_as_uint(sc.light0_b.y), rec.p, r.y, r.z);
+#else
+        const uint32_t li = sc.n_lights > 1 ? min(sc.n_lights - 1u, (uint32_t)(u01(r.w) * (float)sc.n_lights)) : 0u;
+        nd = light_random(sc, __ldg(&sc.lights[li]), rec.p, r.y, r.z, r.w * 0x9E3779B1u);
+#endif
+    } else {
+        const float3 c = random_cosine_direction(u01(r.y), u01(r.z));
+#if !VK_STRICT
+        const Onb uvw = onb_from_w(rec.normal);
+#endif
+        nd = uvw.u * c.x + uvw.v * c.y + uvw.w * c.z;
+    }
+    const float3 und = unit_vector(nd);
+    const float cos_w = dot3(und, onb_w);
+    const float cosine_pdf = cos_w <= 0.0f ? 0.0f : cos_w / VK_PI;
+    const float pdf = 0.5f * lights_pdf_value(sc, rec.p, nd) + 0.5f * cosine_pdf;
+    float spdf = 0.0f;
+    if (spdf_type == VK_M_LAMBERTIAN || spdf_type == VK_M_ISOTROPIC) {
+        const float cos_n = dot3(rec.normal, und);
+        spdf = cos_n < 0.0f ? 0.0f : cos_n / VK_PI;
+    }
+#if VK_STRICT
+    const float3 w = f3(attenuation.x * spdf / pdf, attenuation.y * spdf / pdf, attenuation.z * spdf / pdf);
+#else
+    const float3 w = attenuation * (spdf / pdf);
+#endif
+    if (!finite3(w)) {
+        valid = false;
+        return false;
+    }
+    beta = beta * w;
+    if (beta.x == 0.0f && beta.y == 0.0f && beta.z == 0.0f) return false;
+    o = rec.p;
+    d = nd;
+    return true;
+}
 template <class XI>
 VKD bool shade_xi(const DScene& sc, const HitRecD& rec, const XI& xi, float3& o, float3& d, float& time,
                   float3& beta, float3& L, bool& valid) {
     uint4 m = rec.m;
     uint32_t type = m.x;
     uint32_t spdf_type = type;
-    float3 emitted = f3(0.0f, 0.0f, 0.0f);
     if (!VK_SIMPLE && !VK_LIGHT0 && type == VK_M_SPECDIFFUSE) {
         const uint32_t diffuse = m.w & ~VKD_MAT_NEEDS_UV;
         spdf_type = __ldg(&sc.materials[diffuse]).x;
         m = __ldg(&sc.materials[u01(xi.spec()) < __uint_as_float(m.z) ? m.y : diffuse]);
         type = m.x;
+        if (type == VK_M_DIFFUSE_LIGHT) {
+            L = L + beta * f3(0.0f, 0.0f, 0.0f);
+            return false;
+        }
     } else if (type == VK_M_DIFFUSE_LIGHT) {
-        if (rec.front) emitted = tex_value(sc, m.y, rec.u, rec.v, rec.p);
-    }
-    if (type == VK_M_DIFFUSE_LIGHT) {
-        L = L + beta * emitted;
-        return false;
+        return shade_emitter(sc, rec, m, beta, L);
     }
     const uint4 r = xi.block0();
-    if (type == VK_M_DIELECTRIC) {
-        const float ref_idx = __uint_as_float(m.z);
-        const float etai_over_etat = rec.front ? 1.0f / ref_idx : ref_idx;
-        const float3 unit_direction = unit_vector(d);
-        const float cos_theta = fminf(dot3(-unit_direction, rec.normal), 1.0f);
-        const float sin_theta = sqrtf(1.0f - cos_theta * cos_theta);
-        float3 nd;
-        if (etai_over_etat * sin_theta > 1.0f) nd = reflect(unit_direction, rec.normal);
-        else if (u01(r.x) < schlick(cos_theta, etai_over_etat)) nd = reflect(unit_direction, rec.normal);
-        else nd = refract(unit_direction, rec.normal, etai_over_etat);
-        o = rec.p;
-        d = nd;
-        return true;
-    }
+    if (type == VK_M_DIELECTRIC) return shade_dielectric(rec, m, r, o, d);
     if (!VK_SIMPLE && type == VK_M_METAL) {
         const float fuzz = __uint_as_float(m.z);
         float3 nd = reflect(unit_vector(d), rec.normal);
@@ -1453,51 +1545,7 @@
         time = 0.0f;
         return true;
     }
-    const float3 attenuation = tex_value(sc, m.y, rec.u, rec.v, rec.p);
-#if VK_STRICT
-    const Onb uvw = onb_from_w(rec.normal);
-    const float3 onb_w = uvw.w;
-#else
-    const float3 onb_w = unit_vector(rec.normal);
-#endif
-    float3 nd;
-    if (u01(r.x) < 0.5f) {
-#if VK_SIMPLE || VK_LIGHT0
-        nd = rect_random(sc.light0_a, sc.light0_b.x, __float_as_uint(sc.light0_b.y), rec.p, r.y, r.z);
-#else
-        const uint32_t li = sc.n_lights > 1 ? min(sc.n_lights - 1u, (uint32_t)(u01(r.w) * (float)sc.n_lights)) : 0u;
-        nd = light_random(sc, __ldg(&sc.lights[li]), rec.p, r.y, r.z, r.w * 0x9E3779B1u);
-#endif
-    } else {
-        const float3 c = random_cosine_direction(u01(r.y), u01(r.z));
-#if !VK_STRICT
-        const Onb uvw = onb_from_w(rec.normal);
-#endif
-        nd = uvw.u * c.x + uvw.v * c.y + uvw.w * c.z;
-    }
-    const float3 und = unit_vector(nd);
-    const float cos_w = dot3(und, onb_w);
-    const float cosine_pdf = cos_w <= 0.0f ? 0.0f : cos_w / VK_PI;
-    const float pdf = 0.5f * lights_pdf_value(sc, rec.p, nd) + 0.5f * cosine_pdf;
-    float spdf = 0.0f;
-    if (spdf_type == VK_M_LAMBERTIAN || spdf_type == VK_M_ISOTROPIC) {
-        const float cos_n = dot3(rec.normal, und);
-        spdf = cos_n < 0.0f ? 0.0f : cos_n / VK_PI;
-    }
-#if VK_STRICT
-    const float3 w = f3(attenuation.x * spdf / pdf, attenuation.y * spdf / pdf, attenuation.z * spdf / pdf);
-#else
-    const float3 w = attenuation * (spdf / pdf);
-#endif
-    if (!finite3(w)) {
-        valid = false;
-        return false;
-    }
-    beta = beta * w;
-    if (beta.x == 0.0f && beta.y == 0.0f && beta.z == 0.0f) return false;
-    o = rec.p;
-    d = nd;
-    return true;
+    return shade_diffuse(sc, rec, m, spdf_type, r, o, d, beta, valid);
 }
 VKD bool shade(const DScene& sc, const HitRecD& rec, const PathRng& rng, uint32_t depth, float3& o, float3& d, float& time,
                float3& beta, float3& L, bool& valid) {
diff --git a/vecchio_b200/csrc/vk_internal.h b/vecchio_b200/csrc/vk_internal.h
--- a/vecchio_b200/csrc/vk_internal.h
+++ b/vecchio_b200/csrc/vk_internal.h
@@ -109,6 +109,27 @@
     uint8_t seg_fm0[VKF_MAX_SEGS];
 };
 
+template <int X0, int X1, int Y0, int Y1, int Z0, int Z1, int S0, int S1, int B0, int B1>
+struct FlatSegShape {
+    static constexpr int x0 = X0, x1 = X1, y0 = Y0, y1 = Y1, z0 = Z0, z1 = Z1, s0 = S0, s1 = S1, b0 = B0, b1 = B1;
+    static bool matches(const FlatSeg& g) {
+        auto same = [](uint32_t a0, uint32_t a1, int w0, int w1) { return a1 - a0 == (uint32_t)(w1 - w0) && (w1 == w0 || a0 == (uint32_t)w0); };
+        return same(g.rect0[0], g.rect1[0], X0, X1) && same(g.rect0[1], g.rect1[1], Y0, Y1) && same(g.rect0[2], g.rect1[2], Z0, Z1) &&
+               same(g.sph0, g.sph1, S0, S1) && same(g.box0, g.box1, B0, B1) && g.msph0 == g.msph1 && g.med0 == g.med1 && g.bvh0 == g.bvh1;
+    }
+};
+template <class... Seg>
+struct FlatShape {
+    static constexpr uint32_t n_segs = sizeof...(Seg);
+    static bool matches(const FlatProgram& P) {
+        uint32_t s = 0;
+        return n_segs != 0 && P.n != 0 && P.n_segs == n_segs && P.n_bvh == 0 && (Seg::matches(P.segs[s++]) && ...);
+    }
+};
+using FlatShapeCornell = FlatShape<FlatSegShape<0, 1, 1, 4, 4, 6, 0, 1, 0, 0>, FlatSegShape<0, 0, 0, 0, 0, 0, 0, 0, 0, 1>>;
+enum { VKF_SHAPE_NONE = 0, VKF_SHAPE_CORNELL = 1 };
+inline uint32_t flat_static_shape(const FlatProgram& P) { return FlatShapeCornell::matches(P) ? (uint32_t)VKF_SHAPE_CORNELL : (uint32_t)VKF_SHAPE_NONE; }
+
 struct DCamera {
     float3 origin, lower_left_corner, horizontal, vertical, u, v;
     float lens_radius, time0, time1;
@@ -189,9 +210,9 @@
     cudaError_t launch_staged(const DScene& sc, const FlatProgram* flat, const DCamera& cam, const RenderArgs& a,      \
                               const RenderBuffers& b, unsigned long long* unit_head, int sm_count, cudaStream_t st);   \
     template <class D>                                                                                                 \
-    cudaError_t launch_warpq(const DScene& sc, const FlatProgram* flat, const DCamera& cam, const RenderArgs& a,       \
-                             const RenderBuffers& b, unsigned long long* unit_head, int sm_count, bool legacy,         \
-                             cudaStream_t st, const D& dom);                                                           \
+    cudaError_t launch_warpq(const DScene& sc, const FlatProgram* flat, uint32_t flat_shape, const DCamera& cam,       \
+                             const RenderArgs& a, const RenderBuffers& b, unsigned long long* unit_head, int sm_count, \
+                             bool legacy, cudaStream_t st, const D& dom);                                              \
     size_t stepq_stack_words(uint32_t stack_need, bool inst, int sm_count, uint32_t* levels);                          \
     template <class D>                                                                                                 \
     cudaError_t launch_stepq(const DScene& sc, const DCamera& cam, const RenderArgs& a, const RenderBuffers& b,        \
@@ -210,6 +231,6 @@
 cudaError_t launch_staged(const DScene& sc, const FlatProgram* flat, const DCamera& cam, const RenderArgs& a, const RenderBuffers& b,
                           unsigned long long* unit_head, int sm_count, cudaStream_t st);
 template <class D>
-cudaError_t launch_warpq(const DScene& sc, const FlatProgram* flat, const DCamera& cam, const RenderArgs& a, const RenderBuffers& b,
-                         unsigned long long* unit_head, int sm_count, bool legacy, cudaStream_t st, const D& dom);
+cudaError_t launch_warpq(const DScene& sc, const FlatProgram* flat, uint32_t flat_shape, const DCamera& cam, const RenderArgs& a,
+                         const RenderBuffers& b, unsigned long long* unit_head, int sm_count, bool legacy, cudaStream_t st, const D& dom);
 }
diff --git a/vecchio_b200/csrc/vk_relayout.cu b/vecchio_b200/csrc/vk_relayout.cu
--- a/vecchio_b200/csrc/vk_relayout.cu
+++ b/vecchio_b200/csrc/vk_relayout.cu
@@ -30,6 +30,7 @@
         info->dynamic_megakernel = d->n_nodes >= 65536u ? 1u : 0u;
         info->flat_boxes = 0;
         for (uint32_t s = 0; R.flat.n && s < R.flat.n_segs; ++s) info->flat_boxes += R.flat.segs[s].box1 - R.flat.segs[s].box0;
+        info->flat_shape = R.flat_shape;
         info->flat_direct = 0;
         for (size_t h = 0; 2 * h + 1 < R.flat_shade.size(); ++h) info->flat_direct += __float_as_uint_host(R.flat_shade[2 * h].w) & 1u;
     }
diff --git a/vecchio_b200/csrc/vk_relayout.h b/vecchio_b200/csrc/vk_relayout.h
--- a/vecchio_b200/csrc/vk_relayout.h
+++ b/vecchio_b200/csrc/vk_relayout.h
@@ -489,6 +489,7 @@
     FlatProgram flat{};
     uint32_t levels_world = 0, levels_sub = 0, n_wide = 0, stack_need = 0;
     bool simple = false, has_specdiffuse = false;
+    uint32_t flat_shape = VKF_SHAPE_NONE;
     std::vector<float4> flat_shade;
     std::vector<float4> media_plan;
     const char* run(const vk_scene_desc* d) {
@@ -640,6 +641,7 @@
                 flat_shade[2 * h + 1].x = __uint_as_float_host(mat);
             }
         }
+        flat_shape = flat_static_shape(flat);
         has_specdiffuse = false;
         for (uint32_t i = 0; i < d->n_materials; ++i) has_specdiffuse |= d->materials[i].type == VK_M_SPECDIFFUSE;
         simple = d->n_mspheres == 0 && d->n_lights == 1 && VK_REF_TYPE(d->lights[0]) == VK_T_RECT &&
diff --git a/vecchio_b200/csrc/vk_warpq.cu b/vecchio_b200/csrc/vk_warpq.cu
--- a/vecchio_b200/csrc/vk_warpq.cu
+++ b/vecchio_b200/csrc/vk_warpq.cu
@@ -2,7 +2,10 @@
 
 namespace VK_NS {
 
-template <bool MEDIA, bool LEGACY, class W, int K, bool HYBRID, class D>
+#ifndef VKQ_CLASS_SHADE
+#define VKQ_CLASS_SHADE 1
+#endif
+template <bool MEDIA, bool LEGACY, class W, int K, bool HYBRID, class D, class SHAPE = FlatShape<>>
 VKD void warpq_flat_body(const DScene& sc, const FlatProgram* flat, const DCamera& cam, const RenderArgs& a, const RenderBuffers& buf,
                          unsigned long long* unit_head, const D& dom) {
     extern __shared__ __align__(16) unsigned char vkq_raw[];
@@ -21,7 +24,8 @@
         if (!wq_pick(S, wq_counts(S), EXT_CAP, q, n_q, tail_q)) break;
         const uint32_t n = wq_pop(S, q, n_q, tail_q, q == VKQ_EXT ? EXT_CAP : 32u, lane, head);
         if (q != VKQ_EXT) {
-            wq_shade_batch<LEGACY, !HYBRID>(sc, C, dom, buf, q, n, head, n_drop);
+            constexpr bool SPLIT = VKQ_CLASS_SHADE && SHAPE::n_segs != 0;
+            wq_shade_batch<LEGACY, !HYBRID, SPLIT>(sc, C, dom, buf, q, n, head, n_drop);
             continue;
         }
         wq_converge();
@@ -47,7 +51,13 @@
             if (MEDIA) dom_slot_rng(dom, a, xi[k].rng);
         }
         TraceHit sub[K];
-        trace_flat_k<K, MEDIA, HYBRID>(sc, *flat, o, d, tm, live, 0.001f, xi, best_t, best_hit, sub, &tc);
+#if !VK_STRICT
+        if constexpr (SHAPE::n_segs != 0) {
+            static_assert(!MEDIA && !HYBRID, "a compiled shape has no media and no subtrees");
+            trace_flat_static<K>(*flat, SHAPE{}, o, d, 0.001f, best_t, best_hit);
+        } else
+#endif
+            trace_flat_k<K, MEDIA, HYBRID>(sc, *flat, o, d, tm, live, 0.001f, xi, best_t, best_hit, sub, &tc);
 #pragma unroll
         for (int k = 0; k < K; ++k) {
             uint32_t cls = VKQ_NONE;
@@ -191,6 +201,14 @@
                                                                           const __grid_constant__ D dom) {
     warpq_flat_body<false, LEGACY, WqFlat, VKQ_K_FLAT, false>(sc, &flat, cam, a, buf, unit_head, dom);
 }
+#if VK_SIMPLE
+template <class SHAPE, class D>
+__global__ void __launch_bounds__(32 * VKQ_WARPS, VKQ_MINB_FLAT) k_warpq_flat_static(const DScene sc, const __grid_constant__ FlatProgram flat,
+                                                                                 const DCamera cam, const RenderArgs a, const RenderBuffers buf,
+                                                                                 unsigned long long* unit_head, const __grid_constant__ D dom) {
+    warpq_flat_body<false, false, WqFlat, VKQ_K_FLAT, false, D, SHAPE>(sc, &flat, cam, a, buf, unit_head, dom);
+}
+#endif
 template <bool LEGACY, class D>
 __global__ void __launch_bounds__(32 * VKQ_WARPS, VKQ_MINB_MEDIA) k_warpq_flat_media(const DScene sc, const __grid_constant__ FlatProgram flat,
                                                                                  const DCamera cam, const RenderArgs a, const RenderBuffers buf,
@@ -207,8 +225,8 @@
 #endif
 
 template <class D>
-cudaError_t launch_warpq(const DScene& sc, const FlatProgram* flat, const DCamera& cam, const RenderArgs& a, const RenderBuffers& b,
-                         unsigned long long* unit_head, int sm_count, bool legacy, cudaStream_t st, const D& dom) {
+cudaError_t launch_warpq(const DScene& sc, const FlatProgram* flat, uint32_t flat_shape, const DCamera& cam, const RenderArgs& a,
+                         const RenderBuffers& b, unsigned long long* unit_head, int sm_count, bool legacy, cudaStream_t st, const D& dom) {
     int bps = 0;
     cudaError_t e;
     const bool media = sc.has_media != 0u;
@@ -226,8 +244,11 @@
     }
 #if VK_SIMPLE
     (void)legacy;
-    if (media) VKQ_LAUNCH_FLAT((k_warpq_flat_media<false, D>), WqMedia) else VKQ_LAUNCH_FLAT((k_warpq_flat<false, D>), WqFlat)
+    if (media) VKQ_LAUNCH_FLAT((k_warpq_flat_media<false, D>), WqMedia)
+    else if (flat_shape == VKF_SHAPE_CORNELL) VKQ_LAUNCH_FLAT((k_warpq_flat_static<FlatShapeCornell, D>), WqFlat)
+    else VKQ_LAUNCH_FLAT((k_warpq_flat<false, D>), WqFlat)
 #else
+    (void)flat_shape;
 #define VKQ_LAUNCH_HYB(M, G) VKQ_LAUNCH_FLAT((k_warpq_hybrid<M, G, D>), WqHyb)
     if (flat && flat->n && flat->n_bvh) {
         if (media) { if (legacy) VKQ_LAUNCH_HYB(true, true) else VKQ_LAUNCH_HYB(true, false) }
@@ -246,8 +267,8 @@
     return cudaGetLastError();
 }
 #define VKQ_INSTANTIATE(D)                                                                                             \
-    template cudaError_t launch_warpq(const DScene&, const FlatProgram*, const DCamera&, const RenderArgs&, const RenderBuffers&, \
-                                      unsigned long long*, int, bool, cudaStream_t, const D&);
+    template cudaError_t launch_warpq(const DScene&, const FlatProgram*, uint32_t, const DCamera&, const RenderArgs&,         \
+                                      const RenderBuffers&, unsigned long long*, int, bool, cudaStream_t, const D&);
 VKQ_INSTANTIATE(OneFrame)
 VKQ_INSTANTIATE(FrameArgs)
 VKQ_INSTANTIATE(ListArgs)
diff --git a/vecchio_b200/csrc/vk_warpq.cuh b/vecchio_b200/csrc/vk_warpq.cuh
--- a/vecchio_b200/csrc/vk_warpq.cuh
+++ b/vecchio_b200/csrc/vk_warpq.cuh
@@ -302,86 +302,113 @@
 #ifndef VKQ_FAST_RESOLVE
 #define VKQ_FAST_RESOLVE 1
 #endif
-template <bool LEGACY, bool FLAT, class W, class D>
+template <bool LEGACY, bool FLAT, int CLS, class W, class D>
+VKD void wq_shade_slot(const DScene& sc, const WqCtx<W>& C, const D& dom, const RenderBuffers& buf, bool act, uint32_t slot, bool& alive,
+                       bool& ended, uint32_t& n_drop) {
+    static_assert(CLS == VKQ_NQ || (!LEGACY && (CLS == VKQ_EMIT || CLS == VKQ_DIEL || CLS == VKQ_DIFF)),
+                  "class bodies: the HEAD integrator's emitter, dielectric and diffuse");
+    W& S = C.S;
+    const RenderArgs& a = C.a;
+    if (act) {
+        const float4 ro = S.ro[slot], rd = S.rd[slot], bt = S.bt[slot];
+        const uint4 hp = S.hp[slot];
+        float3 o = f3(ro), d = f3(rd), beta = f3(bt), L = f3(0.0f, 0.0f, 0.0f);
+        float time = ro.w;
+        uint32_t depth = __float_as_uint(rd.w);
+        const uint32_t pixel = S.px[slot], prim = hp.y;
+        bool valid = true;
+#if VKQ_SELFCHECK
+        if (CLS != VKQ_NQ && CLS != VKQ_EMIT && prim == VK_REF_NONE) atomicAdd(&buf.counters[5], 1ull);
+#endif
+        if ((CLS == VKQ_NQ || CLS == VKQ_EMIT) && prim == VK_REF_NONE) {
+            L = beta * miss_color(a, d);
+        } else {
+            PathRng rng;
+            rng.pixel = pixel;
+            rng.sample = __float_as_uint(bt.w);
+            rng.key = make_uint2(a.seed_lo, a.seed_hi);
+            dom_slot_rng(dom, a, rng);
+            HitRecD rec;
+            bool direct = false;
+            uint32_t leaf = prim, hi = hp.z;
+            if (FLAT) {
+                const float4 fs1 = __ldg(&sc.flat_shade[2u * hp.w + 1u]);
+                leaf = __float_as_uint(fs1.y);
+                hi = __float_as_uint(fs1.z);
+#if VKQ_FAST_RESOLVE && !VK_STRICT
+                const float4 fs = __ldg(&sc.flat_shade[2u * hp.w]);
+                const uint32_t fl = __float_as_uint(fs.w);
+                if (fl & 1u) {
+                    direct = true;
+                    const float3 nw = f3(fs);
+                    const bool toward = dot3(d, nw) < 0.0f;
+                    rec.t = __uint_as_float(hp.x);
+                    rec.p = at(o, d, rec.t);
+                    rec.normal = toward ? nw : -nw;
+                    rec.front = (toward ? 1u : 0u) ^ ((fl >> 1) & 1u);
+                    rec.u = 0.0f;
+                    rec.v = 0.0f;
+                    rec.mat = __float_as_uint(fs1.x);
+                    rec.m = __ldg(&sc.materials[rec.mat]);
+                }
+#endif
+            }
+            if (!direct) {
+                TraceHit h;
+                h.t = __uint_as_float(hp.x);
+                h.prim = leaf;
+                h.inst = (hi & 0x80000000u) ? (((uint32_t)VK_T_XFORM << 28) | (hi & 0x07FFFFFFu)) : 0u;
+                h.face = (hi >> 28) & 7u;
+                resolve_hit(sc, h, o, d, time, false, rec);
+            }
+            if constexpr (CLS == VKQ_NQ) {
+                alive = LEGACY ? shade_legacy(sc, rec, rng, depth, o, d, time, beta, L, valid)
+                               : shade(sc, rec, rng, depth, o, d, time, beta, L, valid);
+            } else {
+#if VKQ_SELFCHECK
+                const uint32_t t = rec.m.x;
+                const uint32_t mc = t == VK_M_DIFFUSE_LIGHT ? VKQ_EMIT : t == VK_M_DIELECTRIC ? VKQ_DIEL
+                                  : (t == VK_M_LAMBERTIAN || t == VK_M_ISOTROPIC) ? VKQ_DIFF : VKQ_NONE;
+                if (mc != (uint32_t)CLS) atomicAdd(&buf.counters[5], 1ull);
+#endif
+                if constexpr (CLS == VKQ_EMIT) {
+                    alive = shade_emitter(sc, rec, rec.m, beta, L);
+                } else {
+                    const uint4 r = rng.block(depth, 0u);
+                    if constexpr (CLS == VKQ_DIEL) alive = shade_dielectric(rec, rec.m, r, o, d);
+                    else alive = shade_diffuse(sc, rec, rec.m, rec.m.x, r, o, d, beta, valid);
+                }
+            }
+            if (alive && ++depth > a.max_depth) alive = false;
+            if (alive && !(finite3(d) && finite3(o))) {
+                valid = false;
+                alive = false;
+            }
+        }
+        if (alive) {
+            S.ro[slot] = make_float4(o.x, o.y, o.z, time);
+            S.rd[slot] = make_float4(d.x, d.y, d.z, __uint_as_float(depth));
+            S.bt[slot] = make_float4(beta.x, beta.y, beta.z, bt.w);
+            S.mark_new(slot);
+        } else {
+            if (valid && finite3(L)) dom_accumulate(dom, buf, pixel, L);
+            else ++n_drop;
+            ended = true;
+        }
+    }
+}
+template <bool LEGACY, bool FLAT, bool SPLIT = false, class W, class D>
 VKD void wq_shade_batch(const DScene& sc, const WqCtx<W>& C, const D& dom, const RenderBuffers& buf, uint32_t q, uint32_t n, uint32_t head, uint32_t& n_drop) {
     W& S = C.S;
-    const RenderArgs& a = C.a;
     const uint32_t lane = C.lane;
     const bool act = lane < n;
     const uint32_t slot = S.ring[q][(head + (act ? lane : 0u)) & W::RMASK];
     bool alive = false, ended = false;
-    if (q != VKQ_END) {
-        if (act) {
-            const float4 ro = S.ro[slot], rd = S.rd[slot], bt = S.bt[slot];
-            const uint4 hp = S.hp[slot];
-            float3 o = f3(ro), d = f3(rd), beta = f3(bt), L = f3(0.0f, 0.0f, 0.0f);
-            float time = ro.w;
-            uint32_t depth = __float_as_uint(rd.w);
-            const uint32_t pixel = S.px[slot], prim = hp.y;
-            bool valid = true;
-            if (prim == VK_REF_NONE) {
-                L = beta * miss_color(a, d);
-            } else {
-                PathRng rng;
-                rng.pixel = pixel;
-                rng.sample = __float_as_uint(bt.w);
-                rng.key = make_uint2(a.seed_lo, a.seed_hi);
-                dom_slot_rng(dom, a, rng);
-                HitRecD rec;
-                bool direct = false;
-                uint32_t leaf = prim, hi = hp.z;
-                if (FLAT) {
-                    const float4 fs1 = __ldg(&sc.flat_shade[2u * hp.w + 1u]);
-                    leaf = __float_as_uint(fs1.y);
-                    hi = __float_as_uint(fs1.z);
-#if VKQ_FAST_RESOLVE && !VK_STRICT
-                    const float4 fs = __ldg(&sc.flat_shade[2u * hp.w]);
-                    const uint32_t fl = __float_as_uint(fs.w);
-                    if (fl & 1u) {
-                        direct = true;
-                        const float3 nw = f3(fs);
-                        const bool toward = dot3(d, nw) < 0.0f;
-                        rec.t = __uint_as_float(hp.x);
-                        rec.p = at(o, d, rec.t);
-                        rec.normal = toward ? nw : -nw;
-                        rec.front = (toward ? 1u : 0u) ^ ((fl >> 1) & 1u);
-                        rec.u = 0.0f;
-                        rec.v = 0.0f;
-                        rec.mat = __float_as_uint(fs1.x);
-                        rec.m = __ldg(&sc.materials[rec.mat]);
-                    }
-#endif
-                }
-                if (!direct) {
-                    TraceHit h;
-                    h.t = __uint_as_float(hp.x);
-                    h.prim = leaf;
-                    h.inst = (hi & 0x80000000u) ? (((uint32_t)VK_T_XFORM << 28) | (hi & 0x07FFFFFFu)) : 0u;
-                    h.face = (hi >> 28) & 7u;
-                    resolve_hit(sc, h, o, d, time, false, rec);
-                }
-                alive = LEGACY ? shade_legacy(sc, rec, rng, depth, o, d, time, beta, L, valid)
-                               : shade(sc, rec, rng, depth, o, d, time, beta, L, valid);
-                if (alive && ++depth > a.max_depth) alive = false;
-                if (alive && !(finite3(d) && finite3(o))) {
-                    valid = false;
-                    alive = false;
-                }
-            }
-            if (alive) {
-                S.ro[slot] = make_float4(o.x, o.y, o.z, time);
-                S.rd[slot] = make_float4(d.x, d.y, d.z, __uint_as_float(depth));
-                S.bt[slot] = make_float4(beta.x, beta.y, beta.z, bt.w);
-                S.mark_new(slot);
-            } else {
-                if (valid && finite3(L)) dom_accumulate(dom, buf, pixel, L);
-                else ++n_drop;
-                ended = true;
-            }
-        }
-    } else {
-        ended = act;
-    }
+    if (q == VKQ_END) ended = act;
+    else if constexpr (!SPLIT) wq_shade_slot<LEGACY, FLAT, VKQ_NQ>(sc, C, dom, buf, act, slot, alive, ended, n_drop);
+    else if (q == VKQ_DIFF || q == VKQ_DIFFI) wq_shade_slot<LEGACY, FLAT, VKQ_DIFF>(sc, C, dom, buf, act, slot, alive, ended, n_drop);
+    else if (q == VKQ_EMIT) wq_shade_slot<LEGACY, FLAT, VKQ_EMIT>(sc, C, dom, buf, act, slot, alive, ended, n_drop);
+    else wq_shade_slot<LEGACY, FLAT, VKQ_DIEL>(sc, C, dom, buf, act, slot, alive, ended, n_drop);
     const uint32_t m_end = __ballot_sync(0xFFFFFFFFu, ended);
     bool to_end = false;
     if (q == VKQ_END || (uint32_t)__popc(m_end) >= VKQ_REGEN_MIN) alive = wq_regen(C, dom, ended, slot) || alive;
```

After: 13300, median of 6. 14.7% higher.
